# youthHan/HVRNet

Measured on AMD Instinct MI355X. Metric: VID frames/sec, R101 Faster-RCNN+HVR, 1000x600, 300 props, T=15, higher is better.
Workload: dtype bf16; 1 GPU; configs[2]: faster_rcnn_r101_hrnmp_c5 inference, clip mode; frames_per_window=15, proposals_per_frame=300, input=3x600x1000 padded to 608x1008, parallelism=dp1 independent clips, no collectives, windows_in_flight=4, clips_per_graph=1, key_frame_detections=300

## Files before the change

### hvrnet_amd/csrc/bigtile.hip

```cpp
#include <cstdlib>
#include <type_traits>
#include "common.h"
#include "gemm_params.h"

namespace hvr {

namespace {

constexpr int BG_BN = 256, BG_NT = 512, BG_WN = 4, BG_FN = 4, BG_WCOLS = BG_FN * 16;
constexpr int BG_B_SLOTS = BG_BN * 8 / BG_NT;

__device__ __forceinline__ uint32_t bg_lds_off(const void* p) {
  return (uint32_t)(uintptr_t)(const __attribute__((address_space(3))) char*)p;
}
template <int OFF> __device__ __forceinline__ uint4 bg_read128(uint32_t addr) {
  uint4 v;
  asm volatile("ds_read_b128 %0, %1 offset:%2" : "=v"(v) : "v"(addr), "n"(OFF));
  return v;
}
template <typename T> __device__ __forceinline__ void bg_mma(const uint4& w, const uint4& x, f32x4& acc) {
  if constexpr (std::is_same<T, bf16_t>::value)
    acc = __builtin_amdgcn_mfma_f32_16x16x32_bf16(__builtin_bit_cast(bf16x8, w), __builtin_bit_cast(bf16x8, x), acc, 0, 0, 0);
  else
    acc = __builtin_amdgcn_mfma_f32_16x16x32_f16(__builtin_bit_cast(f16x8, w), __builtin_bit_cast(f16x8, x), acc, 0, 0, 0);
}
__device__ __forceinline__ void bg_load_lds16(const void* base, char* lds, unsigned voff, int soff) {
#if defined(__HIP_DEVICE_COMPILE__)
  const __amdgpu_buffer_rsrc_t rs = __builtin_amdgcn_make_buffer_rsrc(const_cast<void*>(base), 0, (int)0x80000000u, 0x00020000);
  __builtin_amdgcn_raw_ptr_buffer_load_lds(rs, (__attribute__((address_space(3))) void*)lds, 16, (int)voff, soff, 0, 0);
#else
  (void)base; (void)lds; (void)voff; (void)soff;
#endif
}

}

template <typename T, int FM0, int FM1>
__global__ __launch_bounds__(BG_NT) void big_tile_kernel(const GemmParams p) {
  constexpr bool SPLIT = std::is_same<T, f16s_t>::value;
  constexpr int EB = (int)sizeof(T), KSG = 128;
  constexpr int BKE = SPLIT ? 32 : 64;
  constexpr int BM = (FM0 + FM1) * 16;
  constexpr int A_BYTES = BM * 128, STAGE = A_BYTES + BG_BN * 128;
  constexpr int A_SLOTS = (BM * 8 + BG_NT - 1) / BG_NT;
  constexpr int LAST_WAVES = (BM * 8 - (A_SLOTS - 1) * BG_NT) / 64;
  extern __shared__ __attribute__((aligned(16))) char smem[];
  const int tid = threadIdx.x, lane = tid & 63;
  const int wave = __builtin_amdgcn_readfirstlane(tid >> 6);
  const int wm = wave / BG_WN, wn = wave % BG_WN;
  const int wrow0 = wm ? FM0 * 16 : 0;
  const int tiles_n = p.N / BG_BN, tiles_m = (p.M + BM - 1) / BM;
  const int total = tiles_m * tiles_n, nwg = (int)gridDim.x;
  auto tile_of = [&](int r) -> int {
    const int left = total - r * nwg, here = left < nwg ? left : nwg;
    return (int)blockIdx.x < here ? r * nwg + xcd_remap(blockIdx.x, here) : -1;
  };
#ifdef HVR_DBG_BG_CLK
  long long dbg_t[1 + 3 * 3];
  for (int q = 0; q < 10; ++q) dbg_t[q] = 0;
  dbg_t[0] = wall_clock64();
#endif

  const int l_row = tid >> 3, l_chunk = ((tid & 7) ^ (l_row & 7)) * 16;
  int a_bias = 0;
  if (p.conv) a_bias = (int)(((long)p.pad * p.W + p.pad) * p.Cin * EB);
  const char* const rs_a = (const char*)p.A - a_bias;
  const char* const rs_b = (const char*)p.B;
  const bool seg2 = p.s2 > 0;
  const int k1_steps = seg2 ? p.K1 / BKE : 0x7fffffff;
  const char* const rs_a2 = (const char*)p.A2;
  const bool is_conv = p.conv != 0;
  const int cCin = is_conv ? p.Cin : 0x40000000, cKW = is_conv ? p.KW : 1, cDil = is_conv ? p.dil : 0;
  const int cRowB = is_conv ? p.W * p.Cin * EB : 0, cPixB = is_conv ? p.Cin * EB : 0;

  constexpr bool SEG2 = !SPLIT;
  struct TileState { int a_off[A_SLOTS], a_off2[SEG2 ? A_SLOTS : 1], b_off[BG_B_SLOTS]; unsigned oob[A_SLOTS]; int m0, n0; };
  auto setup = [&](int tile, TileState& st) {
    const __attribute__((address_space(4))) GemmParams* kq =
        (const __attribute__((address_space(4))) GemmParams*)__builtin_amdgcn_kernarg_segment_ptr();
    asm volatile("" : "+s"(kq));
    const int pid_m = tile / tiles_n, pid_n = tile - pid_m * tiles_n;
    st.m0 = pid_m * BM;
    st.n0 = pid_n * BG_BN;
    int a_yx[A_SLOTS];
#pragma unroll
    for (int i = 0; i < A_SLOTS; ++i) {
      int m = st.m0 + i * 64 + l_row;
      m = m < kq->M ? m : kq->M - 1;
      if constexpr (SEG2) st.a_off2[i] = 0;
      if (kq->conv || (SEG2 && kq->s2 > 0)) {
        const int ox = m % kq->OW, t = m / kq->OW, oy = t % kq->OH, b = t / kq->OH;
        if (kq->conv) {
          const int iy = oy * kq->stride - kq->pad, ix = ox * kq->stride - kq->pad;
          a_yx[i] = (iy << 16) | (ix & 0xffff);
          st.a_off[i] = (int)((((long)b * kq->H + iy) * kq->W + ix) * (long)kq->Cin * EB) + l_chunk + (int)(((long)kq->pad * kq->W + kq->pad) * kq->Cin * EB);
        } else {
          a_yx[i] = 0;
          st.a_off[i] = (int)((long)m * kq->lda * EB) + l_chunk;
        }
        if constexpr (SEG2) if (kq->s2 > 0) st.a_off2[i] = (int)((((long)b * kq->H2 + oy * kq->s2) * kq->W2 + ox * kq->s2) * (long)(kq->K - kq->K1) * EB) + l_chunk;
      } else {
        a_yx[i] = 0;
        st.a_off[i] = (int)((long)m * kq->lda * EB) + l_chunk;
      }
    }
#pragma unroll
    for (int i = 0; i < BG_B_SLOTS; ++i) st.b_off[i] = (int)((long)(st.n0 + i * 64 + l_row) * kq->ldb * EB) + l_chunk;
#pragma unroll
    for (int i = 0; i < A_SLOTS; ++i) st.oob[i] = 0u;
    if (kq->conv != 0) {
      unsigned colbad[A_SLOTS];
#pragma unroll
      for (int i = 0; i < A_SLOTS; ++i) colbad[i] = 0u;
      for (int kx = 0, dx = 0; kx < kq->KW; ++kx, dx += kq->dil) {
#pragma unroll
        for (int i = 0; i < A_SLOTS; ++i) colbad[i] |= (unsigned)((short)a_yx[i] + dx) < (unsigned)kq->W ? 0u : (1u << kx);
      }
      const unsigned all_kw = kq->KW >= 32 ? ~0u : (1u << kq->KW) - 1u;
      for (int ky = 0, dy = 0, sh = 0; ky < kq->KH; ++ky, dy += kq->dil, sh += kq->KW) {
#pragma unroll
        for (int i = 0; i < A_SLOTS; ++i) st.oob[i] |= ((unsigned)((a_yx[i] >> 16) + dy) < (unsigned)kq->H ? colbad[i] : all_kw) << sh;
      }
    }
  };
  TileState cs, ns;
  int cur_tile = tile_of(0), nxt_tile = tile_of(1);
  setup(cur_tile, cs);
  setup(nxt_tile >= 0 ? nxt_tile : cur_tile, ns);

  int a_koff = 0, b_koff = 0, kt_load = 0, t_cin0 = 0, t_kx = 0, t_ky = 0, t_tap = 0;
  const int nk_real = p.K / BKE;
  auto tap_next = [&](int adv, bool rst) {
    kt_load += adv;
    b_koff += adv * KSG;
    t_cin0 += adv * BKE;
    const bool w1 = t_cin0 >= cCin;
    t_cin0 = w1 ? 0 : t_cin0;
    t_tap += w1 ? 1 : 0;
    t_kx += w1 ? 1 : 0;
    const bool w2 = t_kx >= cKW;
    t_kx = w2 ? 0 : t_kx;
    t_ky += w2 ? 1 : 0;
    const int wmask = -(int)w1;
    a_koff = ((t_ky * cDil * cRowB + t_kx * cDil * cPixB) & wmask) | ((a_koff + adv * KSG) & ~wmask);
    const int keep = rst ? 0 : -1;
    kt_load &= keep; b_koff &= keep; t_cin0 &= keep; t_kx &= keep; t_ky &= keep; t_tap &= keep; a_koff &= keep;
  };
  auto dma_a = [&](auto I, char* stage, bool nx) {
    constexpr int i = decltype(I)::value;
    if (i < A_SLOTS - 1 || wave < LAST_WAVES) {
      const unsigned ao = (unsigned)(nx ? ns.a_off[i] : cs.a_off[i]), ob = nx ? ns.oob[i] : cs.oob[i];
      const unsigned voff = ao | ((ob >> (t_tap & 31)) << 31);
      if constexpr (SEG2) {
        const bool s2 = kt_load >= k1_steps;
        const char* const base = s2 ? rs_a2 : rs_a;
        const unsigned vo = s2 ? (unsigned)(nx ? ns.a_off2[i] : cs.a_off2[i]) : voff;
        const int so = s2 ? (kt_load - k1_steps) * KSG : a_koff;
        bg_load_lds16(base, stage + (i * BG_NT + wave * 64) * 16, vo, __builtin_amdgcn_readfirstlane(so));
      } else {
        bg_load_lds16(rs_a, stage + (i * BG_NT + wave * 64) * 16, voff, __builtin_amdgcn_readfirstlane(a_koff));
      }
    }
  };
  auto dma_b = [&](auto I, char* stage, bool nx) {
    constexpr int i = decltype(I)::value;
    bg_load_lds16(rs_b, stage + A_BYTES + (i * BG_NT + wave * 64) * 16, (unsigned)(nx ? ns.b_off[i] : cs.b_off[i]), __builtin_amdgcn_readfirstlane(b_koff));
  };

  static_for<A_SLOTS>([&](auto I) { dma_a(I, smem, false); });
  static_for<BG_B_SLOTS>([&](auto I) { dma_b(I, smem, false); });

  auto body = [&](auto FMC) {
  constexpr int FM = decltype(FMC)::value;
  int par = 0;
  for (int round = 0;; ++round) {
  const bool has_next = nxt_tile >= 0;
  const int m0 = cs.m0, n0 = cs.n0;
  f32x4 acc[FM][BG_FN];
#pragma unroll
  for (int i = 0; i < FM; ++i)
#pragma unroll
    for (int j = 0; j < BG_FN; ++j) acc[i][j] = f32x4{0.f, 0.f, 0.f, 0.f};

  const int frag_row = lane & 15, frag_grp = lane >> 4, swz = lane & 7;
  const uint32_t a_lane = bg_lds_off(smem) + (wrow0 + frag_row) * 128 + ((frag_grp ^ swz) * 16);
  const uint32_t b_lane = bg_lds_off(smem) + A_BYTES + (wn * BG_WCOLS + frag_row) * 128 + ((frag_grp ^ swz) * 16);

  const int nk = nk_real;
  if (round == 0) asm volatile("s_waitcnt vmcnt(0)" ::: "memory");
  __builtin_amdgcn_s_barrier();
#ifdef HVR_DBG_BG_CLK
  if (round < 3) dbg_t[1 + 3 * round] = wall_clock64();
#endif

  {
    constexpr int G0 = (FM + 1) / 2;
    constexpr int DMA_TOTAL = A_SLOTS + BG_B_SLOTS, DMA_FIRST = DMA_TOTAL / 2;
    auto kloop = [&](auto WMC) __attribute__((always_inline)) {
    constexpr int wmc = decltype(WMC)::value;
    constexpr int dma_ph = wmc ? 0 : 1;
    if constexpr (wmc != 0) __builtin_amdgcn_s_barrier();
    for (int kt = 0; kt < nk; ++kt) {
      const uint32_t soff = (uint32_t)((kt + par) & 1) * STAGE;
      char* nxt = smem + ((kt + 1 + par) & 1) * STAGE;
      const uint32_t a0 = a_lane + soff, b0 = b_lane + soff;
      uint4 kb[BG_FN], qa[G0];
      const bool last = kt + 1 >= nk, pre = last && has_next;
      tap_next(last ? 0 : 1, pre);
      constexpr int NPH = SPLIT ? 6 : 4;
      static_for<NPH>([&](auto PH) {
        constexpr int ph = decltype(PH)::value, term = ph >> 1, r0 = (ph & 1) ? G0 : 0, nr = (ph & 1) ? FM - G0 : G0;
        constexpr bool b_lo = term == 1, a_lo = SPLIT ? term == 2 : term == 1;
        if constexpr ((ph & 1) == 0)
          static_for<BG_FN>([&](auto J) { kb[decltype(J)::value] = bg_read128<decltype(J)::value * 2048>(b_lo ? (b0 ^ 64u) : b0); });
        static_for<nr>([&](auto R) {
          constexpr int r = decltype(R)::value;
          qa[r] = bg_read128<(r0 + r) * 2048>(a_lo ? (a0 ^ 64u) : a0);
        });
        __builtin_amdgcn_sched_barrier(0);
        if constexpr (ph < 3) {
          if constexpr (dma_ph == ph) {
            static_for<DMA_FIRST>([&](auto D) {
              constexpr int d = decltype(D)::value;
              if constexpr (d < A_SLOTS) dma_a(std::integral_constant<int, d>{}, nxt, pre);
              else dma_b(std::integral_constant<int, d - A_SLOTS>{}, nxt, pre);
            });
          } else if constexpr (dma_ph + 1 == ph) {
            static_for<DMA_TOTAL - DMA_FIRST>([&](auto D) {
              constexpr int d = DMA_FIRST + decltype(D)::value;
              if constexpr (d < A_SLOTS) dma_a(std::integral_constant<int, d>{}, nxt, pre);
              else dma_b(std::integral_constant<int, d - A_SLOTS>{}, nxt, pre);
            });
          }
        }
        if constexpr (ph == NPH - 1) {
          if constexpr (wmc != 0) asm volatile("s_waitcnt vmcnt(0)" ::: "memory");
        }
        __builtin_amdgcn_sched_barrier(0);
        __builtin_amdgcn_s_barrier();
        asm volatile("s_waitcnt lgkmcnt(0)" ::: "memory");
        __builtin_amdgcn_sched_barrier(0);
        __builtin_amdgcn_s_setprio(1);
        static_for<nr>([&](auto R) {
          constexpr int r = decltype(R)::value;
          static_for<BG_FN>([&](auto J) { bg_mma<T>(kb[decltype(J)::value], qa[r], acc[r0 + r][decltype(J)::value]); });
        });
        __builtin_amdgcn_s_setprio(0);
        __builtin_amdgcn_sched_barrier(0);
        if constexpr (ph == NPH - 1) {
          if constexpr (wmc == 0) asm volatile("s_waitcnt vmcnt(0)" ::: "memory");
        }
        __builtin_amdgcn_s_barrier();
      });
    }
    if constexpr (wmc == 0) __builtin_amdgcn_s_barrier();
    };
    int wsel = wave;
    asm volatile("" : "+s"(wsel));
    if (wsel >= BG_WN) kloop(std::integral_constant<int, 1>{});
    else kloop(std::integral_constant<int, 0>{});
  }
#ifdef HVR_DBG_BG_CLK
  if (round < 3) dbg_t[2 + 3 * round] = wall_clock64();
#endif

  char* const epi_base = smem + ((nk - 1 + par) & 1) * STAGE;
  const __attribute__((address_space(4))) GemmParams* kp =
      (const __attribute__((address_space(4))) GemmParams*)__builtin_amdgcn_kernarg_segment_ptr();
  asm volatile("" : "+s"(kp));
  if constexpr (SPLIT) {
    int etid = threadIdx.x;
    asm volatile("" : "+v"(etid));
    const int el = etid & 63, erow = el & 15, egrp = el >> 4;
    constexpr int SP = 256;
    char* stg = epi_base + wave * (16 * SP);
    float bias[BG_FN][4];
#pragma unroll
    for (int j = 0; j < BG_FN; ++j) {
      const int n = n0 + wn * BG_WCOLS + j * 16 + egrp * 4;
      if (kp->bias) {
        const float4 b = *reinterpret_cast<const float4*>(kp->bias + n);
        bias[j][0] = b.x; bias[j][1] = b.y; bias[j][2] = b.z; bias[j][3] = b.w;
        if (kp->beta != 0.f) {
#pragma unroll
          for (int r = 0; r < 4; ++r) bias[j][r] *= kp->beta;
        }
      } else {
        bias[j][0] = bias[j][1] = bias[j][2] = bias[j][3] = 0.f;
      }
    }
    auto slot = [&](int j, int plane) {
      const int piece = (j >> 1) * 8 + plane * 4 + 2 * (j & 1) + (egrp >> 1);
      return stg + erow * SP + ((piece ^ erow) << 4) + (egrp & 1) * 8;
    };
    const bool has_res = kp->resid != nullptr;
    const long col_bytes = split_col_bytes(n0 + wn * BG_WCOLS);
    auto load_res = [&](int i, uint4 (&rv)[4]) {
#pragma unroll
      for (int it = 0; it < 4; ++it) {
        const int q = it * 64 + el, row = q >> 4, pc = q & 15;
        int m = m0 + wrow0 + i * 16 + row;
        m = m < kp->M ? m : kp->M - 1;
        rv[it] = *reinterpret_cast<const uint4*>((const char*)kp->resid + (long)m * kp->ldr * 4 + col_bytes + pc * 16);
      }
    };
    uint4 rnext[4] = {make_uint4(0u, 0u, 0u, 0u), make_uint4(0u, 0u, 0u, 0u), make_uint4(0u, 0u, 0u, 0u), make_uint4(0u, 0u, 0u, 0u)};
    if (has_res) load_res(0, rnext);
    asm volatile("s_waitcnt lgkmcnt(0)" ::: "memory");
    __builtin_amdgcn_s_barrier();
#pragma unroll
    for (int i = 0; i < FM; ++i) {
      if (has_res) {
#pragma unroll
        for (int it = 0; it < 4; ++it) {
          const int q = it * 64 + el, row = q >> 4, pc = q & 15;
          *reinterpret_cast<uint4*>(stg + row * SP + ((pc ^ row) << 4)) = rnext[it];
        }
        if (i + 1 < FM) load_res(i + 1, rnext);
      }
#pragma unroll
      for (int j = 0; j < BG_FN; ++j) {
        f32x4 v = acc[i][j];
        if (kp->alpha != 0.f) v *= kp->alpha;
        float e[4];
#pragma unroll
        for (int r = 0; r < 4; ++r) e[r] = v[r] + bias[j][r];
        char* sh = slot(j, 0);
        char* sl = slot(j, 1);
        if (has_res) {
          const uint2 rh = *reinterpret_cast<const uint2*>(sh), rl = *reinterpret_cast<const uint2*>(sl);
          float r0_, r1_, r2_, r3_;
          merge2(rh.x, rl.x, r0_, r1_);
          merge2(rh.y, rl.y, r2_, r3_);
          e[0] += r0_; e[1] += r1_; e[2] += r2_; e[3] += r3_;
        }
        if (kp->relu) {
#pragma unroll
          for (int r = 0; r < 4; ++r) e[r] = fmaxf(e[r], 0.f);
        }
        uint2 oh, ol;
        split2(e[0], e[1], oh.x, ol.x);
        split2(e[2], e[3], oh.y, ol.y);
        *reinterpret_cast<uint2*>(sh) = oh;
        *reinterpret_cast<uint2*>(sl) = ol;
      }
#pragma unroll
      for (int it = 0; it < 4; ++it) {
        const int q = it * 64 + el, row = q >> 4, pc = q & 15;
        const int m = m0 + wrow0 + i * 16 + row;
        const uint4 v = *reinterpret_cast<const uint4*>(stg + row * SP + ((pc ^ row) << 4));
        if (m < kp->M) *reinterpret_cast<uint4*>((char*)kp->C + (long)m * kp->ldc * 4 + col_bytes + pc * 16) = v;
      }
    }
  } else
  {
    int etid = threadIdx.x;
    asm volatile("" : "+v"(etid));
    const int el = etid & 63, erow = el & 15, egrp = el >> 4;
    constexpr int SPITCH = BG_WCOLS * 2;
    char* stg = epi_base + wave * (16 * SPITCH);
    const int wr_lane = erow * SPITCH + (((egrp & 1) ^ (erow >> 3)) << 3);
    float bias[BG_FN][4];
#pragma unroll
    for (int j = 0; j < BG_FN; ++j) {
      const int n = n0 + wn * BG_WCOLS + j * 16 + egrp * 4;
      if (kp->bias) {
        const float4 b = *reinterpret_cast<const float4*>(kp->bias + n);
        bias[j][0] = b.x; bias[j][1] = b.y; bias[j][2] = b.z; bias[j][3] = b.w;
      } else {
        bias[j][0] = bias[j][1] = bias[j][2] = bias[j][3] = 0.f;
      }
    }
    const int st_row = el >> 3, st_chunk = el & 7;
    const bool has_res = kp->resid != nullptr;
    auto load_res = [&](int i, uint4 (&rv)[2]) {
#pragma unroll
      for (int h = 0; h < 2; ++h) {
        int m = m0 + wrow0 + i * 16 + h * 8 + st_row;
        m = m < kp->M ? m : kp->M - 1;
        rv[h] = *reinterpret_cast<const uint4*>((const unsigned short*)kp->resid + (long)m * kp->ldr + n0 + wn * BG_WCOLS + st_chunk * 8);
      }
    };
    uint4 rnext[2] = {make_uint4(0u, 0u, 0u, 0u), make_uint4(0u, 0u, 0u, 0u)};
    if (has_res) load_res(0, rnext);
    asm volatile("s_waitcnt lgkmcnt(0)" ::: "memory");
    __builtin_amdgcn_s_barrier();
#pragma unroll
    for (int i = 0; i < FM; ++i) {
      if (has_res) {
#pragma unroll
        for (int h = 0; h < 2; ++h) {
          const uint4 v = h ? make_uint4(rnext[h].z, rnext[h].w, rnext[h].x, rnext[h].y) : rnext[h];
          *reinterpret_cast<uint4*>(stg + (h * 8 + st_row) * SPITCH + ((st_chunk ^ st_row) << 4)) = v;
        }
        if (i + 1 < FM) load_res(i + 1, rnext);
      }
#pragma unroll
      for (int j = 0; j < BG_FN; ++j) {
        char* slot = stg + wr_lane + (((2 * j + (egrp >> 1)) ^ (erow & 7)) << 4);
        float e[4];
#pragma unroll
        for (int r = 0; r < 4; ++r) e[r] = acc[i][j][r] + bias[j][r];
        if (has_res) {
          const uint2 rr = *reinterpret_cast<const uint2*>(slot);
          float r0_, r1_, r2_, r3_;
          unpack2<T>(rr.x, r0_, r1_);
          unpack2<T>(rr.y, r2_, r3_);
          e[0] += r0_; e[1] += r1_; e[2] += r2_; e[3] += r3_;
        }
        if (kp->relu) {
#pragma unroll
          for (int r = 0; r < 4; ++r) e[r] = fmaxf(e[r], 0.f);
        }
        *reinterpret_cast<uint2*>(slot) = make_uint2(pack2<T>(e[0], e[1]), pack2<T>(e[2], e[3]));
      }
#pragma unroll
      for (int h = 0; h < 2; ++h) {
        const int row = h * 8 + st_row, m = m0 + wrow0 + i * 16 + row;
        uint4 v = *reinterpret_cast<const uint4*>(stg + row * SPITCH + ((st_chunk ^ st_row) << 4));
        if (h) v = make_uint4(v.z, v.w, v.x, v.y);
        if (m < kp->M) *reinterpret_cast<uint4*>((unsigned short*)kp->C + (long)m * kp->ldc + n0 + wn * BG_WCOLS + st_chunk * 8) = v;
      }
    }
  }
#ifdef HVR_DBG_BG_CLK
  if (round < 3) dbg_t[3 + 3 * round] = wall_clock64();
#endif
  if (!has_next) break;
  par = (par + nk) & 1;
  cs = ns;
  cur_tile = nxt_tile;
  nxt_tile = tile_of(round + 2);
  if (nxt_tile >= 0) setup(nxt_tile, ns);
  }
#ifdef HVR_DBG_BG_CLK
  asm volatile("s_waitcnt vmcnt(0)" ::: "memory");
  {
    const long long t_end = wall_clock64();
    if (threadIdx.x == 0 && (blockIdx.x % 5) == 0)
      printf("BGCLK wg %d t0 %lld | tile0 loop %lld..%lld epi %lld | tile1 loop %lld..%lld epi %lld | tile2 loop %lld..%lld epi %lld | drained %lld\n", (int)blockIdx.x, dbg_t[0],
             dbg_t[1] ? dbg_t[1] - dbg_t[0] : 0, dbg_t[2] ? dbg_t[2] - dbg_t[0] : 0, dbg_t[3] ? dbg_t[3] - dbg_t[0] : 0,
             dbg_t[4] ? dbg_t[4] - dbg_t[0] : 0, dbg_t[5] ? dbg_t[5] - dbg_t[0] : 0, dbg_t[6] ? dbg_t[6] - dbg_t[0] : 0,
             dbg_t[7] ? dbg_t[7] - dbg_t[0] : 0, dbg_t[8] ? dbg_t[8] - dbg_t[0] : 0, dbg_t[9] ? dbg_t[9] - dbg_t[0] : 0, t_end - dbg_t[0]);
  }
#endif
  };
  if constexpr (FM0 == FM1) {
    body(std::integral_constant<int, FM0>{});
  } else {
    if (wm == 0) body(std::integral_constant<int, FM0>{});
    else body(std::integral_constant<int, FM1>{});
  }
}

bool bigtile_supported(const GemmParams& p, bool throughput) {
  const bool split = p.dtype == DT_F16S;
  if ((p.dtype != DT_BF16 && p.dtype != DT_F16 && !split) || !p.staging || p.out_f32 || p.ksplit_steps > 0) return false;
  const int es = split ? 4 : 2, bke = split ? 32 : 64, row_al = split ? 32 : 8;
  if (p.s2 > 0 && (split || p.conv || p.K1 % 64 || (p.K - p.K1) % 64 || p.K1 < 64 || (reinterpret_cast<uintptr_t>(p.A2) & 15) ||
                   (long)p.M * (p.K - p.K1) * 2 >= (1L << 31))) return false;
  if (p.N % BG_BN || p.K % bke || p.ldc % row_al || p.lda % row_al || p.ldb % row_al) return false;
  if (p.resid && (p.ldr % row_al || (reinterpret_cast<uintptr_t>(p.resid) & (split ? 127 : 15)))) return false;
  if (split && ((reinterpret_cast<uintptr_t>(p.A) | reinterpret_cast<uintptr_t>(p.B) | reinterpret_cast<uintptr_t>(p.C)) & 127)) return false;
  if (p.tile_hint != kBigForce && (p.K < 256 || (p.resid && throughput && !split))) return false;
  if (p.conv && (p.Cin % bke || p.KH * p.KW > 32)) return false;
  const uintptr_t al = reinterpret_cast<uintptr_t>(p.A) | reinterpret_cast<uintptr_t>(p.B) | reinterpret_cast<uintptr_t>(p.C) |
                       reinterpret_cast<uintptr_t>(p.bias);
  if (al & 15) return false;
  if ((long)p.N * p.ldb * es >= (1L << 31)) return false;
  const long tiles = (long)((p.M + 287) / 288) * (p.N / BG_BN);
  static const int on = std::getenv("HVR_BIGTILE") ? std::atoi(std::getenv("HVR_BIGTILE")) : 1;
  constexpr int min_alone = 170;
  constexpr int min_shared = 96;
  if (p.tile_hint == kBigForce) return true;
  return on && tiles >= (throughput ? min_shared : min_alone) && tiles <= 4096;
}

template <typename T, int FM0, int FM1>
static hipError_t launch_bigtile(const GemmParams& p, hipStream_t stream) {
  constexpr int BM = (FM0 + FM1) * 16, lds = 2 * (BM + BG_BN) * 128;
  auto kern = big_tile_kernel<T, FM0, FM1>;
  static std::atomic<unsigned> attr_set_dev{0};
  per_device_once(attr_set_dev, [&] {
    (void)hipFuncSetAttribute(reinterpret_cast<const void*>(kern), hipFuncAttributeMaxDynamicSharedMemorySize, lds);
  });
  const int tiles = ((p.M + BM - 1) / BM) * (p.N / BG_BN);
  static const int nper = std::getenv("HVR_BIGTILE_WGS") ? std::atoi(std::getenv("HVR_BIGTILE_WGS")) : 256;
  const int grid = nper > 0 && tiles > nper ? nper : tiles;
  hipLaunchKernelGGL(kern, dim3(grid), dim3(BG_NT), lds, stream, p);
  return hipGetLastError();
}

hipError_t run_bigtile(const GemmParams& p, hipStream_t stream) {
  if (p.dtype == DT_F16S) return launch_bigtile<f16s_t, 9, 9>(p, stream);
  if (p.dtype == DT_F16) return launch_bigtile<f16_t, 9, 9>(p, stream);
  return launch_bigtile<bf16_t, 9, 9>(p, stream);
}

}
```

### hvrnet_amd/csrc/capi.hip

```cpp
#include "../../include/hvr_hip.h"

#include <cmath>
#include <cstdarg>
#include <cstdio>
#include <cstdlib>
#include <cstring>
#include <string>

#include "common.h"
#include "gemm_params.h"
#include "relation_bt.h"

namespace hvr {
hipError_t run_transpose_pad(const void*, void*, int, int, long, long, int, hipStream_t);
hipError_t run_zero_fill(void*, size_t, hipStream_t);
hipError_t run_pack_conv_weights_multi(const void*, int, long, int, hipStream_t);
hipError_t run_transpose_multi(const void*, int, int, hipStream_t);
hipError_t run_im2col_t(const void*, void*, int, int, int, int, int, int, int, int, int, int, long, hipStream_t);
hipError_t run_relu_bwd_t(const void*, const void*, void*, void*, int, int, long, hipStream_t);
hipError_t run_splitk_reduce(const float*, float*, int, int, long, int, hipStream_t);
hipError_t run_unpack_conv_wgrads_multi(const void*, int, long, int, hipStream_t);
hipError_t run_splitk_reduce_bf16(const float*, void*, int, int, long, int, hipStream_t);
hipError_t run_splitk_reduce_f16(const float*, void*, int, int, long, int, hipStream_t);
hipError_t run_splitk_reduce_half_batched(const float*, void*, int, int, long, int, int, int, long, long, hipStream_t);
hipError_t run_splitk_reduce_epi_bf16(const float*, void*, int, int, long, int, const float*, const void*, long, int, hipStream_t);
hipError_t run_relation_normalize(void*, const float*, const float*, int, int, long, int, float, hipStream_t);
hipError_t run_relu_bwd(const void*, const void*, void*, long, int, hipStream_t);
hipError_t run_im2col_nhwc(const void*, void*, int, int, int, int, int, int, int, int, int, int, int, hipStream_t);
hipError_t run_scale_rows(const void*, const float*, void*, int, long, int, hipStream_t);
hipError_t run_sgd_step(float*, const float*, float*, long, float, float, float, float, float, float*, int, hipStream_t);
hipError_t run_colsum(const void*, float*, int, int, long, int, float*, hipStream_t);
int colsum_slices(int M, int N);
size_t sgd_workspace_bytes();
hipError_t run_pack_conv_weight(const float*, const float*, void*, int, int, int, int, hipStream_t);
hipError_t run_unpack_conv_wgrad(const float*, const float*, float*, int, int, int, int, hipStream_t);
hipError_t run_det_loss(const float*, int, int, int, int, const long long*, const float*, const float*, const float*, int, float, float,
                        float, float*, float*, const int*, hipStream_t);
size_t assign_workspace_bytes(int n, int k);
hipError_t run_max_iou_assign(const float*, int, int, const float*, int, const uint8_t*, float, float, float, float, long long*, float*,
                              void*, hipStream_t);
hipError_t run_sample(const long long*, const float*, int, int, int, float, long long*, int*, hipStream_t);
hipError_t run_box_targets(const float*, int, int, const float*, const long long*, const long long*, const long long*, const int*, int,
                           const float*, const float*, float, int, long long*, float*, float*, float*, hipStream_t);
hipError_t run_rpn_loss(const float*, int, int, int, const long long*, const float*, const float*, const float*, const int*, float, float*,
                        float*, hipStream_t);
hipError_t run_ce_rows(const float*, int, int, int, const long long*, int, float*, hipStream_t);
hipError_t run_triplet_margin(const void*, long, const void*, long, int, int, int, const long long*, const long long*, const long long*, int,
                              float, int, float*, float*, float*, float*, hipStream_t);
hipError_t run_ingest(const uint8_t*, int, int, long, float*, int, int, int, int, const float*, const float*, int, int, hipStream_t);
size_t tta_merge_proposals_workspace_bytes(int A, int T, int mx);
hipError_t run_tta_merge_proposals(const float*, const int*, int, int, int, const float*, const float*, const int*, float, int, float*, int*, void*,
                                   hipStream_t);
hipError_t run_tta_map_rois(const float*, int, int, int, const float*, const float*, const int*, float*, hipStream_t);
hipError_t run_tta_merge_dets(const float*, const float*, int, int, int, const float*, const float*, const int*, float*, float*, hipStream_t);
hipError_t run_mining_argreduce(const float*, int, int, long, const long long*, const long long*, long long*, hipStream_t);
hipError_t run_relation_dscore(const void*, const void*, const void*, const void*, void*, int, long, int, long, long, float, int, hipStream_t);
hipError_t run_im2col_stem(const float*, void*, int, int, int, int, int, int, int, hipStream_t);
hipError_t run_maxpool3x3s2(const void*, void*, int, int, int, int, int, int, int, hipStream_t);
hipError_t run_cast(const void*, void*, long, int, int, float, hipStream_t);
hipError_t run_permute(const void*, void*, int, int, int, int, int, int, hipStream_t);
hipError_t run_det_decode(const float*, int, int, int, int, const float*, int, const float*, const float*, float, float,
                          float, float, float*, float*, hipStream_t);
hipError_t run_roi_align_fwd(const void*, const float*, void*, int, int, int, int, int, int, int, float, int, int, int,
                             hipStream_t);
hipError_t run_roi_align_bwd(const float*, const float*, float*, int, int, int, int, int, int, float, int, int, hipStream_t);
hipError_t run_deform_im2col(const void*, const float*, void*, int, int, int, int, int, int, int, int, int, int, int, int, long, int, int,
                             hipStream_t);
size_t nms_workspace_bytes(int P, int n);
hipError_t run_nms_batched(const float*, int, int, float, int, int, int, long long*, int*, void*, hipStream_t, int band = 0,
                           int* band_done = nullptr);
hipError_t run_rpn_select(const void*, const void*, long, long, float*, const RpnParams&, int, hipStream_t);
hipError_t run_rpn_select_wide(const void*, const void*, long, long, float*, const RpnParams&, void*, hipStream_t);
size_t rpn_wide_workspace_bytes(int T, long n_anchor);
int rpn_wide_max_frames(int set);
int* rpn_wide_done_flags(void* wws, int T);
hipError_t run_rpn_gather(const float*, const long long*, const int*, int, int, int, int, int, float*, int*, hipStream_t);
hipError_t run_multiclass_nms(const float*, const float*, int, int, float, float, int, float*, long long*, int*, void*,
                              hipStream_t);
size_t multiclass_nms_workspace_bytes(int R, int ncls);
hipError_t run_soft_nms(const float*, int, float, int, float, float, float*, long long*, int*, hipStream_t);
hipError_t run_multiclass_soft_nms(const float*, const float*, int, int, int, float, float, int, float, float, int, float*, long long*, int*,
                                   void*, hipStream_t);
size_t multiclass_soft_nms_workspace_bytes(int P, int R, int ncls);
hipError_t run_seq_nms(const float*, const float*, int, const int*, int, int, int, float, float, float, int, int, float*, long long*, int*, int*,
                       int*, float*, int*, int, void*, int, hipStream_t);
size_t seq_nms_workspace_bytes(int P, int F, int R, int ncls, int tubes);
hipError_t run_stem_fused(const float*, const void*, const float*, void*, int, int, int, int, hipStream_t);
}

using namespace hvr;

static thread_local std::string g_err;

static int fail(int code, const char* fmt, ...) {
  char buf[512];
  va_list ap;
  va_start(ap, fmt);
  vsnprintf(buf, sizeof buf, fmt, ap);
  va_end(ap);
  g_err = buf;
  return code;
}
static int check_launch(hipError_t e, const char* what) {
  if (e == hipSuccess) return HVR_OK;
  if (e == hipErrorInvalidValue) return fail(HVR_EUNSUPPORTED, "%s: shape outside the implemented envelope", what);
  return fail(HVR_ELAUNCH, "%s: %s", what, hipGetErrorString(e));
}
static inline size_t align256(size_t b) { return (b + 255) & ~(size_t)255; }
static inline int elem_size(int dtype) { return (dtype == HVR_BF16 || dtype == HVR_F16) ? 2 : 4; }
static inline int kstep_elems(int dtype) { return (dtype == HVR_F32 || dtype == HVR_F16S) ? 32 : 64; }
static inline bool valid_dtype(int dtype) { return dtype >= HVR_F32 && dtype <= HVR_F16S; }
static inline bool aligned128(const void* p) { return (reinterpret_cast<uintptr_t>(p) & 127) == 0; }
static inline bool aligned16(const void* p) { return (reinterpret_cast<uintptr_t>(p) & 15) == 0; }

extern "C" {

int hvr_abi_version(void) { return 6; }
const char* hvr_last_error(void) { return g_err.c_str(); }

static int fill_linear(GemmParams& p, const void* A, const void* B, void* C, int M, int N, int K, long lda, long ldb,
                       long ldc, int dtype, int staging) {
  std::memset(&p, 0, sizeof p);
  if (!valid_dtype(dtype)) return fail(HVR_EINVAL, "dtype %d is none of HVR_F32 / HVR_BF16 / HVR_F16 / HVR_F16S", dtype);
  const int bke = kstep_elems(dtype);
  if (!A || !B || !C) return fail(HVR_EINVAL, "null operand pointer");
  if (M <= 0 || N <= 0 || K <= 0) return fail(HVR_EINVAL, "empty problem M=%d N=%d K=%d", M, N, K);
  if (K % bke) return fail(HVR_EINVAL, "K=%d is not a multiple of the %d-element K-step", K, bke);
  if (N % 4) return fail(HVR_EINVAL, "N=%d is not a multiple of 4", N);
  if (!aligned16(A) || !aligned16(B) || !aligned16(C)) return fail(HVR_EINVAL, "operands must be 16-byte aligned");
  if (dtype == HVR_F16S && (lda % 32 || ldb % 32 || !aligned128(A) || !aligned128(B)))
    return fail(HVR_EINVAL, "split-half operands need 128-byte aligned bases and row pitches that are multiples of 32 elements");
  const long es = elem_size(dtype);
  if ((long)M * lda * es >= (1L << 31) || (long)N * ldb * es >= (1L << 31))
    return fail(HVR_EUNSUPPORTED, "operand of 2 GiB or more (M=%d lda=%ld N=%d ldb=%ld)", M, lda, N, ldb);
  p.A = A; p.B = B; p.C = C;
  p.M = M; p.N = N; p.K = K;
  p.lda = lda; p.ldb = ldb; p.ldc = ldc;
  p.dtype = dtype;
  p.staging = staging ? 1 : 0;
  return HVR_OK;
}

static int fewrow_mode() {
  static const int on = std::getenv("HVR_CONV_SPLITK") ? std::atoi(std::getenv("HVR_CONV_SPLITK")) : 1;
  return on;
}
static int fewrow_slices(const GemmParams& p) {
  const int on = fewrow_mode();
  constexpr int target = 512, mink = 8, minper = 4;
  if (!on || p.dtype != DT_BF16 || !p.staging || p.out_f32 || p.tile_hint != 0) return 1;
  if (p.N % 8 || p.ldc % 8 || (p.resid && p.ldr % 8) || !aligned16(p.C) || (p.resid && !aligned16(p.resid)) || (p.bias && !aligned16(p.bias))) return 1;
  const long tiles = (long)((p.M + 127) / 128) * ((p.N + 63) / 64);
  const int ksteps = p.K / 64;
  if (tiles > 160 || ksteps < mink) return 1;
  long s = (target + tiles / 2) / tiles;
  if (s > ksteps / minper) s = ksteps / minper;
  return s < 2 ? 1 : (int)s;
}

static hipError_t run_fewrow_split(const GemmParams& p, int slices, void* ws, hipStream_t stream) {
  GemmParams q = p;
  const int ksteps = p.K / 64;
  q.ksplit_steps = (ksteps + slices - 1) / slices;
  q.ksplit_count = (ksteps + q.ksplit_steps - 1) / q.ksplit_steps;
  q.csplit_bytes = (long)p.M * p.N * 4;
  q.C = ws; q.ldc = p.N; q.out_f32 = 1;
  q.bias = nullptr; q.resid = nullptr; q.relu = 0;
  q.tile_hint = 2;
  hipError_t e = run_tile_op(q, EPI_LINEAR, stream);
  if (e == hipSuccess) e = run_splitk_reduce_epi_bf16((const float*)ws, p.C, p.M, p.N, p.ldc, q.ksplit_count, p.bias, p.resid, p.ldr, p.relu, stream);
  return e;
}

static int gemm_params(const hvr_gemm_desc* d, GemmParams& p) {
  if (!d) return fail(HVR_EINVAL, "null descriptor");
  int rc = fill_linear(p, d->A, d->B, d->C, d->M, d->N, d->K, d->lda, d->ldb, d->ldc, d->dtype, d->staging);
  if (rc) return rc;
  const int es = elem_size(d->dtype);
  if ((d->lda * es) % 16 || (d->ldb * es) % 16) return fail(HVR_EINVAL, "lda/ldb rows must be 16-byte multiples");
  if ((d->ldc * (d->out_f32 ? 4 : es)) % 8) return fail(HVR_EINVAL, "ldc rows must be 8-byte multiples");
  if (d->dtype == HVR_F16S) {
    if (!d->out_f32 && (d->N % 8 || d->ldc % 32 || !aligned128(d->C))) return fail(HVR_EINVAL, "split-half output: N %% 8 == 0, ldc %% 32 == 0, 128-byte aligned C");
    if (d->resid && (d->N % 8 || d->ldr % 32 || !aligned128(d->resid))) return fail(HVR_EINVAL, "split-half residual: N %% 8 == 0, ldr %% 32 == 0, 128-byte aligned");
  }
  p.bias = d->bias; p.resid = d->resid; p.ldr = d->ldr; p.relu = d->relu; p.out_f32 = d->out_f32;
  p.tile_hint = d->tile_hint;
  p.alpha = d->alpha; p.beta = d->beta;
  return 0;
}

size_t hvr_gemm_fewrow_workspace_bytes(const hvr_gemm_desc* d) {
  GemmParams p;
  if (gemm_params(d, p)) return 0;
  const int s = fewrow_slices(p);
  return s > 1 ? (size_t)s * p.M * p.N * 4 : 0;
}

int hvr_gemm(const hvr_gemm_desc* d, void* stream) {
  GemmParams p;
  const int rc = gemm_params(d, p);
  if (rc) return rc;
  int hint = d->tile_hint;
  if (hint == kBigForce) {
    if (!bigtile_supported(p, true)) return fail(HVR_EUNSUPPORTED, "the big-tile kernel takes bf16 products with N %% 256 == 0 and K %% 64 == 0");
    return check_launch(run_bigtile(p, (hipStream_t)stream), "hvr_gemm(big tile)");
  }
  if (hint == kBigHint || hint == 0) {
    const bool thr = hint == kBigHint;
    p.tile_hint = hint = 0;
    if (bigtile_supported(p, thr)) return check_launch(run_bigtile(p, (hipStream_t)stream), "hvr_gemm(big tile)");
  }
  if (d->tile_hint == kPcHint128 || d->tile_hint == kPcHint256) {
    if (!pc_supported(p, EPI_LINEAR)) return fail(HVR_EUNSUPPORTED, "the producer / consumer tile kernel takes aligned bf16 operands with N %% 8 == 0");
    return check_launch(run_pc(p, EPI_LINEAR, d->tile_hint == kPcHint256 ? 256 : 128, (hipStream_t)stream), "hvr_gemm (pc)");
  }
  if (hint == 0 && d->K >= 8192 && pc_supported(p, EPI_LINEAR)) {
    const long tiles = (long)((d->M + 143) / 144) * ((d->N + 127) / 128);
    if (tiles > 192 && tiles <= 256) return check_launch(run_pc(p, EPI_LINEAR, 128, (hipStream_t)stream), "hvr_gemm (pc)");
  }
  const int slices = fewrow_slices(p);
  if (slices > 1 && d->ws && aligned16(d->ws) && d->ws_bytes >= (size_t)slices * p.M * p.N * 4) {
    if (fewrow_mode() == 1 && kpar_supported(p)) return check_launch(run_kpar(p, (hipStream_t)stream), "hvr_gemm(K-parallel waves)");
    return check_launch(run_fewrow_split(p, slices, d->ws, (hipStream_t)stream), "hvr_gemm(split-K)");
  }
  return check_launch(run_tile_op(p, EPI_LINEAR, (hipStream_t)stream), "hvr_gemm");
}

static int splitk_slices(int M, int N, int K, int dtype) {
  const long tiles = (long)((M + 127) / 128) * ((N + 127) / 128);
  if (dtype == HVR_F16S) return 1;
  const int ksteps = K / kstep_elems(dtype);
  if (tiles >= 192 || ksteps < 32) return 1;
  long s = (512 + tiles - 1) / tiles;
  if (s > ksteps / 8) s = ksteps / 8;
  if (s > 64) s = 64;
  return s < 2 ? 1 : (int)s;
}

size_t hvr_gemm_splitk_workspace_bytes(int M, int N, int K, int dtype) {
  if (M <= 0 || N <= 0 || K <= 0 || !valid_dtype(dtype)) return 0;
  const int s = splitk_slices(M, N, K, dtype);
  return s > 1 ? (size_t)s * M * N * 4 : 0;
}

int hvr_gemm_splitk(const hvr_gemm_desc* d, void* ws, size_t ws_bytes, void* stream) {
  if (!d) return fail(HVR_EINVAL, "null descriptor");
  if (d->bias || d->resid || d->relu) return fail(HVR_EINVAL, "split-K products have no epilogue (bias / residual / ReLU)");
  if (d->dtype != HVR_F32 && !d->out_f32) return fail(HVR_EINVAL, "split-K products are f32 (set out_f32)");
  GemmParams p;
  int rc = fill_linear(p, d->A, d->B, d->C, d->M, d->N, d->K, d->lda, d->ldb, d->ldc, d->dtype, d->staging);
  if (rc) return rc;
  const int es = elem_size(d->dtype);
  if ((d->lda * es) % 16 || (d->ldb * es) % 16) return fail(HVR_EINVAL, "lda/ldb rows must be 16-byte multiples");
  if ((d->ldc * 4) % 8) return fail(HVR_EINVAL, "ldc rows must be 8-byte multiples");
  p.out_f32 = d->out_f32;
  p.tile_hint = d->tile_hint;
  const int slices = splitk_slices(d->M, d->N, d->K, d->dtype);
  if (slices <= 1) return check_launch(run_tile_op(p, EPI_LINEAR, (hipStream_t)stream), "hvr_gemm_splitk");
  const size_t need = (size_t)slices * d->M * d->N * 4;
  if (!ws || ws_bytes < need || !aligned16(ws)) return fail(HVR_EINVAL, "split-K workspace too small (%zu < %zu) or unaligned", ws_bytes, need);
  const int ksteps = d->K / kstep_elems(d->dtype);
  p.ksplit_steps = (ksteps + slices - 1) / slices;
  p.ksplit_count = (ksteps + p.ksplit_steps - 1) / p.ksplit_steps;
  p.csplit_bytes = (long)d->M * d->N * 4;
  p.C = ws;
  p.ldc = d->N;
  hipError_t e = run_tile_op(p, EPI_LINEAR, (hipStream_t)stream);
  if (e == hipSuccess) e = run_splitk_reduce((const float*)ws, (float*)d->C, d->M, d->N, d->ldc, p.ksplit_count, (hipStream_t)stream);
  return check_launch(e, "hvr_gemm_splitk");
}

static int splitk_slices_batched(int M, int N, int K, int dtype, int count) {
  const long tiles = (long)((M + 127) / 128) * ((N + 127) / 128) * count;
  if (dtype == HVR_F16S) return 1;
  const int ksteps = K / kstep_elems(dtype);
  if (tiles >= 384 || ksteps < 32) return 1;
  long s = (512 + tiles - 1) / tiles;
  if (s > ksteps / 8) s = ksteps / 8;
  if (s > 64) s = 64;
  return s < 2 ? 1 : (int)s;
}

size_t hvr_gemm_splitk_batched_workspace_bytes(int M, int N, int K, int dtype, int count) {
  if (M <= 0 || N <= 0 || K <= 0 || count <= 0 || !valid_dtype(dtype)) return 0;
  const int s = splitk_slices_batched(M, N, K, dtype, count);
  return s > 1 ? (size_t)s * count * M * N * 4 : 0;
}

int hvr_gemm_splitk_batched(const hvr_gemm_desc* d, int count, int64_t stride_a, int64_t stride_b, int64_t stride_c, void* ws, size_t ws_bytes,
                            void* stream) {
  if (!d || count <= 0) return fail(HVR_EINVAL, "null descriptor / count <= 0");
  if (d->bias || d->resid || d->relu) return fail(HVR_EINVAL, "split-K products have no epilogue (bias / residual / ReLU)");
  if (d->dtype != HVR_F32 && !d->out_f32) return fail(HVR_EINVAL, "split-K products are f32 (set out_f32)");
  if (d->dtype == HVR_F16S) return fail(HVR_EUNSUPPORTED, "batched split-K products take f32 / bf16 / half operands");
  GemmParams p;
  int rc = fill_linear(p, d->A, d->B, d->C, d->M, d->N, d->K, d->lda, d->ldb, d->ldc, d->dtype, d->staging);
  if (rc) return rc;
  const int es = elem_size(d->dtype);
  if ((d->lda * es) % 16 || (d->ldb * es) % 16 || (stride_a * es) % 16 || (stride_b * es) % 16) return fail(HVR_EINVAL, "lda / ldb rows and the problem strides must be 16-byte multiples");
  if ((d->ldc * 4) % 8 || (stride_c * 4) % 16) return fail(HVR_EINVAL, "ldc rows must be 8-byte, stride_c 16-byte multiples");
  if (stride_a * es >= (1L << 31) || stride_b * es >= (1L << 31)) return fail(HVR_EUNSUPPORTED, "one problem's operands must stay below 2 GiB");
  p.out_f32 = d->out_f32;
  p.tile_hint = d->tile_hint;
  p.batch = count;
  p.gs_a = stride_a * es; p.gs_b = stride_b * es; p.gs_c = stride_c * 4;
  const int slices = splitk_slices_batched(d->M, d->N, d->K, d->dtype, count);
  if (slices <= 1) return check_launch(run_tile_op(p, EPI_LINEAR, (hipStream_t)stream), "hvr_gemm_splitk_batched");
  if (d->ldc != d->N || stride_c != (int64_t)d->M * d->N) return fail(HVR_EINVAL, "the sliced form writes one contiguous [count][M][N] output (ldc = N, stride_c = M * N)");
  const size_t need = (size_t)slices * count * d->M * d->N * 4;
  if (!ws || ws_bytes < need || !aligned16(ws)) return fail(HVR_EINVAL, "split-K workspace too small (%zu < %zu) or unaligned", ws_bytes, need);
  if ((long)count * d->M > 0x7fffffffL) return fail(HVR_EUNSUPPORTED, "too many output rows");
  const int ksteps = d->K / kstep_elems(d->dtype);
  p.ksplit_steps = (ksteps + slices - 1) / slices;
  p.ksplit_count = (ksteps + p.ksplit_steps - 1) / p.ksplit_steps;
  p.csplit_bytes = (long)count * d->M * d->N * 4;
  p.gs_c = (long)d->M * d->N * 4;
  p.C = ws;
  p.ldc = d->N;
  hipError_t e = run_tile_op(p, EPI_LINEAR, (hipStream_t)stream);
  if (e == hipSuccess) e = run_splitk_reduce((const float*)ws, (float*)d->C, count * d->M, d->N, d->N, p.ksplit_count, (hipStream_t)stream);
  return check_launch(e, "hvr_gemm_splitk_batched");
}

static int expand_enabled() {
  static const int on = std::getenv("HVR_EXPAND") ? std::atoi(std::getenv("HVR_EXPAND")) : 1;
  return on;
}

static int conv_params(const hvr_conv_desc* d, GemmParams& p, int& path) {
  if (!d) return fail(HVR_EINVAL, "null descriptor");
  const int OH = (d->H + 2 * d->pad - d->dil * (d->KH - 1) - 1) / d->stride + 1;
  const int OW = (d->W + 2 * d->pad - d->dil * (d->KW - 1) - 1) / d->stride + 1;
  if (OH <= 0 || OW <= 0) return fail(HVR_EINVAL, "empty conv output %dx%d", OH, OW);
  if (!valid_dtype(d->dtype)) return fail(HVR_EINVAL, "bad dtype %d", d->dtype);
  const int bke = kstep_elems(d->dtype);
  if (d->Cin % bke) return fail(HVR_EINVAL, "Cin=%d is not a multiple of %d", d->Cin, bke);
  if (d->dtype == HVR_F16S && !d->out_f32 && (d->Cout % 32 || !aligned128(d->y))) return fail(HVR_EINVAL, "split-half conv output: Cout %% 32 == 0, 128-byte aligned y");
  if (d->dtype == HVR_F16S && d->resid && (d->Cout % 32 || !aligned128(d->resid))) return fail(HVR_EINVAL, "split-half conv residual: Cout %% 32 == 0, 128-byte aligned");
  const long M = (long)d->B * OH * OW;
  if (M > 0x7fffffffL) return fail(HVR_EUNSUPPORTED, "too many output pixels");
  if ((long)d->B * d->H * d->W * d->Cin * (long)elem_size(d->dtype) >= (1L << 31))
    return fail(HVR_EUNSUPPORTED, "conv input of 2 GiB or more");
  const int K = d->KH * d->KW * d->Cin;
  int rc = fill_linear(p, d->x, d->w, d->y, (int)M, d->Cout, K, d->Cin, K, d->Cout, d->dtype, d->staging);
  if (rc) return rc;
  const bool pointwise = d->KH == 1 && d->KW == 1 && d->stride == 1 && d->pad == 0;
  if (!pointwise) {
    if (!d->zero) return fail(HVR_EINVAL, "conv needs the zero page");
    p.conv = 1; p.H = d->H; p.W = d->W; p.Cin = d->Cin; p.OH = OH; p.OW = OW; p.KH = d->KH; p.KW = d->KW;
    p.stride = d->stride; p.pad = d->pad; p.dil = d->dil; p.zero = d->zero;
  }
  p.bias = d->bias; p.resid = d->resid; p.ldr = d->Cout; p.relu = d->relu; p.out_f32 = d->out_f32;
  p.tile_hint = d->tile_hint;
  p.alpha = d->alpha; p.beta = d->beta;
  if (pointwise) p.zero = d->zero;
  const int use_expand = expand_enabled();
  if (p.tile_hint == kBigForce) {
    path = 0;
    return 0;
  }
  const bool hint0 = p.tile_hint == 0 || p.tile_hint == kBigHint;
  bool big_first = false;
  if (hint0 && pointwise) {
    GemmParams q = p;
    q.tile_hint = 0;
    big_first = bigtile_supported(q, p.tile_hint == kBigHint);
    if (big_first && p.resid && p.K == 256 && p.dtype != DT_F16S && p.M >= 65536 && expand_supported(p)) big_first = false;
  }
  path = (pointwise && (expand_supported(p) || expand_split_supported(p)) &&
          (p.tile_hint == kExpandHint || (hint0 && use_expand && p.resid && p.N >= 2 * p.K && !big_first))) ? 1 : 0;
  if (p.tile_hint == kExpandHint) p.tile_hint = 0;
  static const int use_c3 = std::getenv("HVR_CONV3") ? std::atoi(std::getenv("HVR_CONV3")) : 1;
  if (path == 0 && hint0 && use_c3 && conv3x3_c64_supported(p)) path = 2;
  if (path != 0 && p.tile_hint == kBigHint) p.tile_hint = 0;
  return 0;
}

size_t hvr_conv2d_splitk_workspace_bytes(const hvr_conv_desc* d) {
  GemmParams p;
  int path = 0;
  if (conv_params(d, p, path)) return 0;
  const int s = (path == 0 ? fewrow_slices(p) : 1);
  return s > 1 ? (size_t)s * p.M * p.N * 4 : 0;
}

int hvr_conv2d_nhwc(const hvr_conv_desc* d, void* stream) {
  GemmParams p;
  int path = 0;
  const int rc = conv_params(d, p, path);
  if (rc) return rc;
  if (path == 1) return check_launch(p.dtype == DT_F16S ? run_expand_split(p, (hipStream_t)stream) : run_expand(p, (hipStream_t)stream), "hvr_conv2d_nhwc(expand)");
  if (path == 2) return check_launch(run_conv3x3_c64(p, (hipStream_t)stream), "hvr_conv2d_nhwc(conv3x3_c64)");
  if (path == 0 && d->tile_hint == kBigForce) {
    if (!bigtile_supported(p, true)) return fail(HVR_EUNSUPPORTED, "the big-tile kernel takes bf16 convs with Cout %% 256 == 0 and Cin %% 64 == 0");
    return check_launch(run_bigtile(p, (hipStream_t)stream), "hvr_conv2d_nhwc(big tile)");
  }
  if (path == 0 && d->tile_hint == kTwoLevelHint) {
    p.tile_hint = 0;
    if (two_level_supported(p)) return check_launch(run_tile_op(p, EPI_LINEAR2, (hipStream_t)stream), "hvr_conv2d_nhwc(two-level)");
  }
  if (path == 0 && (d->tile_hint == kBigHint || d->tile_hint == 0 || d->tile_hint == kTwoLevelHint)) {
    p.tile_hint = 0;
    if (bigtile_supported(p, d->tile_hint == kBigHint)) return check_launch(run_bigtile(p, (hipStream_t)stream), "hvr_conv2d_nhwc(big tile)");
  }
  const int slices = (path == 0 ? fewrow_slices(p) : 1);
  if (slices > 1 && d->ws && aligned16(d->ws) && d->ws_bytes >= (size_t)slices * p.M * p.N * 4) {
    if (fewrow_mode() == 1 && kpar_supported(p)) return check_launch(run_kpar(p, (hipStream_t)stream), "hvr_conv2d_nhwc(K-parallel waves)");
    const hipError_t e = run_fewrow_split(p, slices, d->ws, (hipStream_t)stream);
    return check_launch(e, "hvr_conv2d_nhwc(split-K)");
  }
  return check_launch(run_tile_op(p, EPI_LINEAR, (hipStream_t)stream), "hvr_conv2d_nhwc");
}

static int tail_params(const hvr_tail_desc* d, GemmParams& p) {
  if (!d) return fail(HVR_EINVAL, "null descriptor");
  if (d->dtype != HVR_BF16 && d->dtype != HVR_F16) return fail(HVR_EUNSUPPORTED, "hvr_bottleneck_tail takes bf16 or half operands");
  if (d->B <= 0 || d->OH <= 0 || d->OW <= 0 || d->stride2 <= 0) return fail(HVR_EINVAL, "empty tail problem");
  if ((d->OH - 1) * d->stride2 >= d->H2 || (d->OW - 1) * d->stride2 >= d->W2) return fail(HVR_EINVAL, "the sampled pixels fall outside x");
  const long M = (long)d->B * d->OH * d->OW;
  if (M > 0x7fffffffL) return fail(HVR_EUNSUPPORTED, "too many output pixels");
  const int K = d->C1 + d->C2;
  int rc = fill_linear(p, d->h, d->w, d->y, (int)M, d->Cout, K, d->C1, K, d->Cout, d->dtype, 1);
  if (rc) return rc;
  if (!d->x || !aligned16(d->x)) return fail(HVR_EINVAL, "x must be a 16-byte aligned device pointer");
  if ((long)d->B * d->H2 * d->W2 * d->C2 * 2 >= (1L << 31)) return fail(HVR_EUNSUPPORTED, "block input of 2 GiB or more");
  p.bias = d->bias; p.relu = d->relu;
  p.A2 = d->x; p.K1 = d->C1; p.H2 = d->H2; p.W2 = d->W2; p.s2 = d->stride2; p.OH = d->OH; p.OW = d->OW;
  return 0;
}

static bool tail_on_tile_engine(const GemmParams& p) {
  return (p.dtype == DT_BF16 || p.dtype == DT_F16) && p.K1 % 64 == 0 && (p.K - p.K1) % 64 == 0 && p.K1 >= 64 && p.K - p.K1 >= 64 && p.N % 8 == 0 && p.ldc % 8 == 0 &&
         (long)p.M * (p.K - p.K1) * 2 < (1L << 31);
}

int hvr_bottleneck_tail_supported(const hvr_tail_desc* d) {
  GemmParams p;
  if (tail_params(d, p)) return 0;
  return (expand_supported(p) || tail_on_tile_engine(p)) ? 1 : 0;
}

int hvr_bottleneck_tail(const hvr_tail_desc* d, void* stream) {
  GemmParams p;
  const int rc = tail_params(d, p);
  if (rc) return rc;
  if (expand_supported(p)) return check_launch(run_expand(p, (hipStream_t)stream), "hvr_bottleneck_tail");
  if (tail_on_tile_engine(p)) {
    if (bigtile_supported(p, false)) return check_launch(run_bigtile(p, (hipStream_t)stream), "hvr_bottleneck_tail(big tile)");
    return check_launch(run_tile_op(p, EPI_LINEAR, (hipStream_t)stream), "hvr_bottleneck_tail(tile engine)");
  }
  return fail(HVR_EUNSUPPORTED, "no fused tail kernel for C1=%d C2=%d Cout=%d", d->C1, d->C2, d->Cout);
}

static int tail_next_params(const hvr_tail_next_desc* d, GemmParams& p) {
  if (!d) return fail(HVR_EINVAL, "null descriptor");
  const hvr_tail_desc& t = d->tail;
  if (t.C2 > 0) {
    const int rc = tail_params(&t, p);
    if (rc) return rc;
  } else {
    if (t.dtype != HVR_BF16 && t.dtype != HVR_F16 && t.dtype != HVR_F16S)
      return fail(HVR_EUNSUPPORTED, "hvr_bottleneck_tail_next takes bf16, half or (identity form) split-half operands");
    if (t.B <= 0 || t.OH <= 0 || t.OW <= 0) return fail(HVR_EINVAL, "empty tail problem");
    const long M = (long)t.B * t.OH * t.OW;
    if (M > 0x7fffffffL) return fail(HVR_EUNSUPPORTED, "too many output pixels");
    const int rc = fill_linear(p, t.h, t.w, t.y, (int)M, t.Cout, t.C1, t.C1, t.C1, t.Cout, t.dtype, 1);
    if (rc) return rc;
    const bool split = t.dtype == HVR_F16S;
    if (!d->resid || !(split ? aligned128(d->resid) : aligned16(d->resid)))
      return fail(HVR_EINVAL, "an identity block needs its (16-byte aligned; split half: 128-byte aligned) residual map");
    if (split && (t.Cout % 32 || !aligned128(t.y))) return fail(HVR_EINVAL, "split-half tail: Cout %% 32 == 0, 128-byte aligned y");
    p.bias = t.bias; p.relu = t.relu; p.resid = d->resid; p.ldr = t.Cout;
    if (t.dtype == HVR_F16S) { p.alpha = d->alpha; p.beta = d->beta; }
  }
  if (!t.relu) return fail(HVR_EUNSUPPORTED, "the next block reads the activated output (relu = 1)");
  p.Wn = d->wn; p.bias_n = d->bias_n; p.Hn = d->hn; p.Cn = d->Cn;
  return 0;
}

int hvr_bottleneck_tail_next_supported(const hvr_tail_next_desc* d) {
  GemmParams p;
  if (tail_next_params(d, p)) return 0;
  return (expand_next_supported(p) || expand_split_next_supported(p)) ? 1 : 0;
}

int hvr_bottleneck_tail_next(const hvr_tail_next_desc* d, void* stream) {
  GemmParams p;
  const int rc = tail_next_params(d, p);
  if (rc) return rc;
  if (expand_split_next_supported(p)) return check_launch(run_expand_split(p, (hipStream_t)stream), "hvr_bottleneck_tail_next(split half)");
  if (!expand_next_supported(p))
    return fail(HVR_EUNSUPPORTED, "no fused tail + next conv kernel for C1=%d C2=%d Cout=%d Cn=%d", d->tail.C1, d->tail.C2, d->tail.Cout, d->Cn);
  return check_launch(run_expand(p, (hipStream_t)stream), "hvr_bottleneck_tail_next");
}

static int close_sampled_params(const hvr_close_sampled_desc* d, GemmParams& p) {
  if (!d) return fail(HVR_EINVAL, "null descriptor");
  if (!valid_dtype(d->dtype)) return fail(HVR_EINVAL, "bad dtype %d", d->dtype);
  if (d->B <= 0 || d->OH <= 0 || d->OW <= 0 || d->rstride <= 0 || d->RH <= 0 || d->RW <= 0) return fail(HVR_EINVAL, "empty sampled-close problem");
  if ((long)(d->OH - 1) * d->rstride >= d->RH || (long)(d->OW - 1) * d->rstride >= d->RW) return fail(HVR_EINVAL, "the sampled pixels fall outside resid");
  const long M = (long)d->B * d->OH * d->OW;
  if (M > 0x7fffffffL || (long)d->B * d->RH * d->RW > 0x7fffffffL) return fail(HVR_EUNSUPPORTED, "too many pixels");
  const int rc = fill_linear(p, d->h, d->w, d->y, (int)M, d->Cout, d->C1, d->C1, d->C1, d->Cout, d->dtype, 1);
  if (rc) return rc;
  const bool split = d->dtype == HVR_F16S;
  if (!d->resid || !(split ? aligned128(d->resid) : aligned16(d->resid)))
    return fail(HVR_EINVAL, "resid must be a 16-byte aligned (split half: 128-byte aligned) device pointer");
  if (split && (d->Cout % 32 || !aligned128(d->y))) return fail(HVR_EINVAL, "split-half sampled close: Cout %% 32 == 0, 128-byte aligned y");
  p.bias = d->bias; p.relu = d->relu; p.resid = d->resid; p.ldr = d->Cout;
  p.rs = d->rstride; p.RH = d->RH; p.RW = d->RW; p.OH = d->OH; p.OW = d->OW;
  if (split) { p.alpha = d->alpha; p.beta = d->beta; }
  return 0;
}

int hvr_bottleneck_close_sampled_supported(const hvr_close_sampled_desc* d) {
  GemmParams p;
  if (close_sampled_params(d, p)) return 0;
  return (expand_enabled() && p.N >= 2 * p.K && (expand_supported(p) || expand_split_supported(p))) ? 1 : 0;
}

int hvr_bottleneck_close_sampled(const hvr_close_sampled_desc* d, void* stream) {
  GemmParams p;
  const int rc = close_sampled_params(d, p);
  if (rc) return rc;
  if (expand_enabled() && p.N >= 2 * p.K) {
    if (expand_split_supported(p)) return check_launch(run_expand_split(p, (hipStream_t)stream), "hvr_bottleneck_close_sampled(split half)");
    if (expand_supported(p)) return check_launch(run_expand(p, (hipStream_t)stream), "hvr_bottleneck_close_sampled");
  }
  return fail(HVR_EUNSUPPORTED, "no sampled-residual closing kernel for C1=%d Cout=%d dtype=%d (%d output pixels)", d->C1, d->Cout, d->dtype, p.M);
}

int hvr_conv2d_path(const hvr_conv_desc* d) {
  GemmParams p;
  int path = 0;
  const int rc = conv_params(d, p, path);
  if (rc) return rc;
  if (path == 0 && (d->tile_hint == 0 || d->tile_hint == kBigHint)) {
    p.tile_hint = 0;
    if (bigtile_supported(p, d->tile_hint == kBigHint)) return 3;
  }
  return path;
}

int hvr_im2col_stem(const float* img, void* cols, int B, int H, int W, int KP, int dtype, void* stream) {
  if (!img || !cols || B <= 0) return fail(HVR_EINVAL, "bad stem arguments");
  if (dtype == HVR_F16S && (KP % 32 || !aligned128(cols))) return fail(HVR_EINVAL, "split-half patch rows: KP %% 32 == 0, 128-byte aligned");
  if (KP < 147 || KP % kstep_elems(dtype)) return fail(HVR_EINVAL, "KP=%d must be >= 147 and a K-step multiple", KP);
  const int OH = (H + 6 - 7) / 2 + 1, OW = (W + 6 - 7) / 2 + 1;
  return check_launch(run_im2col_stem(img, cols, B, H, W, OH, OW, KP, dtype, (hipStream_t)stream), "hvr_im2col_stem");
}

int hvr_stem_fused_dtype(const float* img, const void* wpk, const float* bias, void* out, int B, int H, int W, int dtype, void* stream) {
  if (!img || !wpk || !bias || !out || B <= 0 || H < 7 || W < 7) return fail(HVR_EINVAL, "bad fused-stem arguments");
  if (dtype != HVR_BF16 && dtype != HVR_F16 && dtype != HVR_F16S) return fail(HVR_EUNSUPPORTED, "the fused stem computes on bf16, half or split-half operands");
  if (!aligned16(wpk) || !aligned16(out) || !aligned16(bias)) return fail(HVR_EINVAL, "fused stem operands must be 16-byte aligned");
  if (dtype == HVR_F16S && !aligned128(out)) return fail(HVR_EINVAL, "split-half stem output must be 128-byte aligned");
  return check_launch(run_stem_fused(img, wpk, bias, out, B, H, W, dtype, (hipStream_t)stream), "hvr_stem_fused");
}
int hvr_stem_fused(const float* img, const void* wpk, const float* bias, void* out, int B, int H, int W, void* stream) {
  return hvr_stem_fused_dtype(img, wpk, bias, out, B, H, W, HVR_BF16, stream);
}

int hvr_maxpool3x3s2_nhwc(const void* x, void* y, int B, int H, int W, int C, int dtype, void* stream) {
  if (!x || !y || C % 4) return fail(HVR_EINVAL, "bad maxpool arguments (C %% 4 == 0 required)");
  if (dtype == HVR_F16S) return fail(HVR_EUNSUPPORTED, "max pooling runs on f32 / bf16 / half maps");
  const int OH = (H + 2 - 3) / 2 + 1, OW = (W + 2 - 3) / 2 + 1;
  return check_launch(run_maxpool3x3s2(x, y, B, H, W, C, OH, OW, dtype, (hipStream_t)stream), "hvr_maxpool3x3s2_nhwc");
}

static int env_tile(const char* name) {
  const char* v = std::getenv(name);
  return v ? std::atoi(v) : 0;
}
static inline long rel_ldp(int Mk) { return ((long)Mk + 127) / 128 * 128; }

static int apply_slice_blocks() { return 4; }
static int apply_slices(int Mq, int Mk, int D) {
  const long tiles = (long)((Mq + 127) / 128) * ((D + 127) / 128);
  const int nblk = (int)(rel_ldp(Mk) / 128);
  if (tiles >= 96 || nblk < 8 || D % 8) return 1;
  const int per = apply_slice_blocks();
  return (nblk + per - 1) / per;
}

static int relation_apply_pass(const void* P, const void* Vt, float* mstat, float* lstat, float* partial, void* O, int64_t ldo,
                               int Mq, int Mk, int D, long ldp, int nt, int dtype, int staging, hipStream_t s) {
  const bool two_byte = dtype == HVR_BF16 || dtype == HVR_F16;
  constexpr int tile_apply = 0, gm_apply = 1;
#ifdef HVR_DEBUG_KNOBS
  static const int dbg_ld0 = env_tile("HVR_DBG_LD0");
#endif
  GemmParams p;
  int rc;
  rc = fill_linear(p, P, Vt, O, Mq, D, (int)ldp, ldp, ldp, ldo, dtype, staging);
  if (rc) return rc;
  p.mstat = mstat; p.lstat = lstat; p.ntile = nt;
  p.tile_hint = tile_apply;
  p.group_m = gm_apply;
#ifdef HVR_DEBUG_KNOBS
  if (dbg_ld0 & 2) { p.lda = 0; p.ldb = 0; }
#endif
  const int slices = apply_slices(Mq, Mk, D);
  if (slices > 1 && tile_apply == 0 && (!two_byte || (ldo % 8 == 0 && aligned16(O)))) {
    const int steps_per_blk = two_byte ? 2 : 4;
    const int per = apply_slice_blocks();
    p.ksplit_steps = per * steps_per_blk;
    p.ksplit_count = slices;
    p.csplit_bytes = (long)Mq * D * 4;
    p.C = partial; p.ldc = D; p.out_f32 = two_byte ? 1 : 0;
    p.tile_hint = 1;
    hipError_t e = run_tile_op(p, EPI_APPLY, s);
    if (e == hipSuccess)
      e = dtype == HVR_BF16 ? run_splitk_reduce_bf16(partial, O, Mq, D, ldo, slices, s)
          : dtype == HVR_F16 ? run_splitk_reduce_f16(partial, O, Mq, D, ldo, slices, s) : run_splitk_reduce(partial, (float*)O, Mq, D, ldo, slices, s);
    return check_launch(e, "relation: apply (key slices)");
  }
  if (Mq >= 1024 && pc_supported(p, EPI_APPLY))
    return check_launch(run_pc(p, EPI_APPLY, 128, s), "relation: apply (pc)");
  return check_launch(run_tile_op(p, EPI_APPLY, s), "relation: apply");
}

constexpr int kNormalizeMaxBlocks = 128;
static int normalize_blocks_ok(int Mk, const char* what) {
  if (rel_ldp(Mk) / 128 > kNormalizeMaxBlocks)
    return fail(HVR_EUNSUPPORTED, "%s: Mk=%d exceeds the %d keys (%d blocks of 128) the normalising sweep supports", what, Mk,
                kNormalizeMaxBlocks * 128, kNormalizeMaxBlocks);
  return HVR_OK;
}
static bool split_normalizes(int Mq) {
  static const int split_normalize = std::getenv("HVR_SPLIT_NORMALIZE") ? std::atoi(std::getenv("HVR_SPLIT_NORMALIZE")) : -1;
  return split_normalize == 1 || (split_normalize < 0 && Mq >= 1024);
}

static int relation_split_tail(void* P, void* Vt, float* mstat, float* lstat, const void* V, int64_t ldv, void* O, int64_t ldo, int Mq,
                               int Mk, int D, long ldp, int nt, int staging, hipStream_t s) {
  constexpr int tile_apply_s = 0;
  int rc = V ? check_launch(run_transpose_pad(V, Vt, Mk, D, ldv, ldp, HVR_F16S, s), "relation: V transpose (split half)") : HVR_OK;
  if (rc) return rc;
  GemmParams p;
  rc = fill_linear(p, P, Vt, O, Mq, D, (int)ldp, ldp, ldp, ldo, HVR_F16S, staging);
  if (rc) return rc;
  p.alpha = 1.f / kSplitProbScale;
  p.mstat = mstat; p.lstat = lstat; p.ntile = nt;
  p.tile_hint = tile_apply_s;
#ifdef HVR_DEBUG_KNOBS
  static const int dbg_apply_s = env_tile("HVR_DBG_APPLY_S");
  if (dbg_apply_s) p.tile_hint = dbg_apply_s;
#endif
  if (split_normalizes(Mq)) {
    rc = check_launch(run_relation_normalize(P, mstat, lstat, Mq, nt, ldp, HVR_F16S, 1.f, s), "relation: normalise (split half)");
    if (rc) return rc;
    return check_launch(run_tile_op(p, EPI_LINEAR, s), "relation: apply (split half, plain product)");
  }
  return check_launch(run_tile_op(p, EPI_APPLY, s), "relation: apply (split half)");
}

size_t hvr_relation_workspace_bytes(int Mq, int Mk, int D, int dtype) {
  const long ldp = rel_ldp(Mk), nt = ldp / 128;
  const size_t es = elem_size(dtype);
  const int slices = apply_slices(Mq, Mk, D);
  return align256((size_t)Mq * ldp * es) + align256((size_t)D * ldp * es) + 2 * align256((size_t)Mq * nt * 4) +
         (slices > 1 ? align256((size_t)slices * Mq * D * 4) : 0);
}

int hvr_relation_fwd(const void* Q, int64_t ldq, const void* K, int64_t ldk, const void* V, int64_t ldv, void* O,
                     int64_t ldo, int Mq, int Mk, int D, float scale, int dtype, int staging, void* ws, size_t ws_bytes,
                     void* stream) {
  if (!Q || !K || !V || !O || !ws) return fail(HVR_EINVAL, "null pointer");
  if (Mq <= 0 || Mk <= 0) return fail(HVR_EINVAL, "empty relation Mq=%d Mk=%d", Mq, Mk);
  if (!(scale > 0.f)) return fail(HVR_EINVAL, "relation scale must be positive (the reference uses 1/sqrt(D)), got %g", (double)scale);
  if (ws_bytes < hvr_relation_workspace_bytes(Mq, Mk, D, dtype))
    return fail(HVR_EWORKSPACE, "relation workspace %zu < %zu", ws_bytes, hvr_relation_workspace_bytes(Mq, Mk, D, dtype));
  const long ldp = rel_ldp(Mk);
  const int nt = (int)(ldp / 128);
  const size_t es = elem_size(dtype);
  char* w = (char*)ws;
  void* P = w;                w += align256((size_t)Mq * ldp * es);
  void* Vt = w;               w += align256((size_t)D * ldp * es);
  float* mstat = (float*)w;   w += align256((size_t)Mq * nt * 4);
  float* lstat = (float*)w;   w += align256((size_t)Mq * nt * 4);
  float* partial = (float*)w;
  hipStream_t s = (hipStream_t)stream;

  GemmParams p;
  int rc;
  constexpr int tile_scores_s = 0;
  if (dtype == HVR_F16S) {
    if (ldv % 64 || !aligned128(V) || ldo % 32 || !aligned128(O) || D % 64) return fail(HVR_EINVAL, "split-half relation: D, ldv multiples of 64, ldo of 32, 128-byte aligned V / O");
    if (split_normalizes(Mq) && (rc = normalize_blocks_ok(Mk, "split-half relation"))) return rc;
    const bool bt = staging && scores_bt_supported(Mq, Mk, D, ldq, ldk, ldv, ldp, Q, K, V, P, Vt, 1, true);
    if (bt) {
      ScoresBTParams b;
      b.Q = (const bf16_t*)Q; b.K = (const bf16_t*)K; b.P = (bf16_t*)P; b.mstat = mstat; b.lstat = lstat;
      b.V = (const bf16_t*)V; b.Vt = (bf16_t*)Vt; b.Mq = Mq; b.Mk = Mk; b.D = D; b.ntile = nt;
      b.ldq = ldq; b.ldk = ldk; b.ldv = ldv; b.ldp = ldp; b.sl2 = scale * 1.4426950408889634f; b.f16 = 2;
      b.groups = 1; b.gs_q = b.gs_k = b.gs_v = b.gs_p = b.gs_vt = b.gs_stat = 0; b.int_max = 0;
      rc = check_launch(run_scores_bt(b, s), "relation: scores (split half, big tile)");
    } else {
      rc = fill_linear(p, Q, K, P, Mq, (Mk + 3) / 4 * 4, D, ldq, ldk, ldp, dtype, staging);
      if (rc) return rc;
      p.N = Mk; p.scale = scale; p.mstat = mstat; p.lstat = lstat; p.ntile = nt; p.group_m = 8;
      p.tile_hint = tile_scores_s;
      rc = check_launch(run_tile_op(p, EPI_SCORES, s), "relation: scores (split half)");
    }
    if (rc) return rc;
    return relation_split_tail(P, Vt, mstat, lstat, bt ? nullptr : V, ldv, O, ldo, Mq, Mk, D, ldp, nt, staging, s);
  }
  const bool two_byte = dtype == HVR_BF16 || dtype == HVR_F16;
  constexpr int tile_scores = 0, gm_scores = 8;
#ifdef HVR_DEBUG_KNOBS
  static const int dbg_ld0 = env_tile("HVR_DBG_LD0");
#endif
  const bool bt = two_byte && staging && scores_bt_supported(Mq, Mk, D, ldq, ldk, ldv, ldp, Q, K, V, P, Vt);
  if (bt) {
    ScoresBTParams b;
    b.Q = (const bf16_t*)Q; b.K = (const bf16_t*)K; b.P = (bf16_t*)P; b.mstat = mstat; b.lstat = lstat;
    b.V = (const bf16_t*)V; b.Vt = (bf16_t*)Vt; b.Mq = Mq; b.Mk = Mk; b.D = D; b.ntile = nt;
    b.ldq = ldq; b.ldk = ldk; b.ldv = ldv; b.ldp = ldp; b.sl2 = scale * 1.4426950408889634f; b.f16 = dtype == HVR_F16;
    b.groups = 1; b.gs_q = b.gs_k = b.gs_v = b.gs_p = b.gs_vt = b.gs_stat = 0; b.int_max = 0;
    rc = check_launch(run_scores_bt(b, s), "relation: scores (big tile)");
    if (rc) return rc;
  } else {
    const bool fold = two_byte && staging && Mq <= 1024 && D % 8 == 0 && ldv % 8 == 0 && aligned16(V) && aligned16(Vt);
    if (!fold) {
      rc = check_launch(run_transpose_pad(V, Vt, Mk, D, ldv, ldp, dtype, s), "relation: V transpose");
      if (rc) return rc;
    }
    rc = fill_linear(p, Q, K, P, Mq, (Mk + 3) / 4 * 4, D, ldq, ldk, ldp, dtype, staging);
    if (rc) return rc;
    if (fold) {
      p.tr_in = V; p.tr_out = Vt; p.tr_R = Mk; p.tr_C = D; p.tr_ldx = ldv; p.tr_ldt = ldp;
      const int score_tiles = ((Mq + 127) / 128) * ((Mk + 127) / 128);
      const int vt_tiles = ((D + 63) / 64) * (int)((ldp + 63) / 64);
      int nb = 256 - score_tiles % 256;
      if (nb < 64) nb += 256;
      p.tr_blocks = nb < vt_tiles ? nb : vt_tiles;
    }
    p.N = Mk;
    p.scale = scale; p.mstat = mstat; p.lstat = lstat; p.ntile = nt;
    p.tile_hint = tile_scores ? tile_scores : ((two_byte && staging && Mq <= 1024) ? 9 : 0);
    p.group_m = gm_scores;
#ifdef HVR_DEBUG_KNOBS
    if (dbg_ld0 & 1) { p.lda = 0; p.ldb = 0; }
#endif
    rc = check_launch(run_tile_op(p, EPI_SCORES, s), "relation: scores");
    if (rc) return rc;
  }
  return relation_apply_pass(P, Vt, mstat, lstat, partial, O, ldo, Mq, Mk, D, ldp, nt, dtype, staging, s);
}

size_t hvr_relation_grouped_workspace_bytes(int groups, int Mq, int Mk, int D, int dtype) {
  return (size_t)(groups > 0 ? groups : 0) * align256(hvr_relation_workspace_bytes(Mq, Mk, D, dtype));
}

// ... 717 lines not shown
```

### hvrnet_amd/csrc/gemm_params.h

```cpp
#pragma once
#include <hip/hip_runtime.h>

namespace hvr {

enum { EPI_LINEAR = 0, EPI_SCORES = 1, EPI_APPLY = 2, EPI_LINEAR2 = 3 };

struct RpnParams {
  int T, H, W, A, npre, n_anchor;
  int cls_pitch, reg_pitch;
  int stride;
  float img_h, img_w;
  float m[4], s[4];
  float max_ratio;
  float base[32][4];
};

struct GemmParams {
  const void* A;
  const void* B;
  void* C;
  int M, N, K;
  long lda, ldb, ldc;
  int dtype;
  int staging;
  int tile_hint;
  int conv, H, W, Cin, OH, OW, KH, KW, stride, pad, dil;
  const void* zero;
  const float* bias;
  const void* resid;
  long ldr;
  int relu, out_f32;
  float alpha;
  float beta;
  float scale;
  float* mstat;
  float* lstat;
  int ntile;
  int group_m;
  const void* A2;
  int K1, H2, W2, s2;
  int rs, RH, RW;
  const void* Wn;
  const float* bias_n;
  void* Hn;
  int Cn;
  int ksplit_steps, ksplit_count;
  long csplit_bytes;
  const void* tr_in;
  void* tr_out;
  int tr_R, tr_C, tr_blocks;
  long tr_ldx, tr_ldt;
  int batch;
  long gs_a, gs_b, gs_c, gs_stat, gs_tr_in, gs_tr_out;
};

struct TileShape { int bm, bn, wg_per_cu; float eff; };
constexpr int kNumTileShapes = 12;
constexpr int kNumBaseShapes = 5;
extern const TileShape kTileShapes[kNumTileShapes];
int choose_tile(const GemmParams& p, int epi);

hipError_t run_tile_op(const GemmParams& p, int epi, hipStream_t stream);
bool two_level_supported(const GemmParams& p);

constexpr int kExpandHint = kNumTileShapes + 1;
bool expand_supported(const GemmParams& p);
bool conv3x3_c64_supported(const GemmParams& p);
hipError_t run_conv3x3_c64(const GemmParams& p, hipStream_t stream);
hipError_t run_expand(const GemmParams& p, hipStream_t stream);
bool expand_next_supported(const GemmParams& p);
bool expand_split_supported(const GemmParams& p);
bool expand_split_next_supported(const GemmParams& p);
hipError_t run_expand_split(const GemmParams& p, hipStream_t stream);
constexpr int kPcHint128 = kNumTileShapes + 2, kPcHint256 = kNumTileShapes + 3;
bool pc_supported(const GemmParams& p, int epi);
constexpr int kBigHint = kNumTileShapes + 4, kBigForce = kNumTileShapes + 5, kTwoLevelHint = kNumTileShapes + 6;
constexpr int kTwoLevelSteps = 8;
bool bigtile_supported(const GemmParams& p, bool throughput);
hipError_t run_bigtile(const GemmParams& p, hipStream_t stream);
hipError_t run_pc(const GemmParams& p, int epi, int bn, hipStream_t stream);
bool kpar_supported(const GemmParams& p);
hipError_t run_kpar(const GemmParams& p, hipStream_t stream);

}
```

### hvrnet_amd/native.py

```python
import contextlib
import ctypes
import math
import os
import subprocess

import torch

_HERE = os.path.dirname(os.path.abspath(__file__))
LIB_PATH = os.path.join(_HERE, 'libhvr_hip.so')
HEADER_PATH = os.path.join(os.path.dirname(_HERE), 'include', 'hvr_hip.h')

HVR_F32, HVR_BF16, HVR_F16, HVR_F16S = 0, 1, 2, 3
ABI_VERSION = 6
SPLIT = torch.int32
COMPUTE_DTYPES = (torch.bfloat16, torch.float16, SPLIT, torch.float32)
DTYPE_NAMES = {torch.bfloat16: 'bf16', torch.float16: 'f16', SPLIT: 'f16x2', torch.float32: 'f32'}
LAYOUT_NCHW, LAYOUT_NHWC = 0, 1

STAGING = 1
TILE_HINT = 0


class HvrError(RuntimeError):
    pass


class GemmDesc(ctypes.Structure):
    _fields_ = [('A', ctypes.c_void_p), ('B', ctypes.c_void_p), ('C', ctypes.c_void_p),
                ('M', ctypes.c_int32), ('N', ctypes.c_int32), ('K', ctypes.c_int32),
                ('lda', ctypes.c_int64), ('ldb', ctypes.c_int64), ('ldc', ctypes.c_int64),
                ('bias', ctypes.c_void_p), ('resid', ctypes.c_void_p), ('ldr', ctypes.c_int64),
                ('relu', ctypes.c_int32), ('out_f32', ctypes.c_int32),
                ('dtype', ctypes.c_int32), ('staging', ctypes.c_int32), ('tile_hint', ctypes.c_int32),
                ('ws', ctypes.c_void_p), ('ws_bytes', ctypes.c_size_t), ('alpha', ctypes.c_float), ('beta', ctypes.c_float)]


class ConvDesc(ctypes.Structure):
    _fields_ = [('x', ctypes.c_void_p), ('w', ctypes.c_void_p), ('y', ctypes.c_void_p),
                ('B', ctypes.c_int32), ('H', ctypes.c_int32), ('W', ctypes.c_int32),
                ('Cin', ctypes.c_int32), ('Cout', ctypes.c_int32), ('KH', ctypes.c_int32),
                ('KW', ctypes.c_int32), ('stride', ctypes.c_int32), ('pad', ctypes.c_int32),
                ('dil', ctypes.c_int32),
                ('bias', ctypes.c_void_p), ('resid', ctypes.c_void_p),
                ('relu', ctypes.c_int32), ('out_f32', ctypes.c_int32),
                ('dtype', ctypes.c_int32), ('staging', ctypes.c_int32), ('tile_hint', ctypes.c_int32),
                ('zero', ctypes.c_void_p), ('ws', ctypes.c_void_p), ('ws_bytes', ctypes.c_size_t), ('alpha', ctypes.c_float),
                ('beta', ctypes.c_float)]


class TailDesc(ctypes.Structure):
    _fields_ = [('h', ctypes.c_void_p), ('x', ctypes.c_void_p), ('w', ctypes.c_void_p), ('y', ctypes.c_void_p),
                ('B', ctypes.c_int32), ('OH', ctypes.c_int32), ('OW', ctypes.c_int32), ('C1', ctypes.c_int32),
                ('H2', ctypes.c_int32), ('W2', ctypes.c_int32), ('C2', ctypes.c_int32), ('stride2', ctypes.c_int32),
                ('Cout', ctypes.c_int32), ('bias', ctypes.c_void_p), ('relu', ctypes.c_int32), ('dtype', ctypes.c_int32)]


class TailNextDesc(ctypes.Structure):
    _fields_ = [('tail', TailDesc), ('resid', ctypes.c_void_p), ('wn', ctypes.c_void_p), ('bias_n', ctypes.c_void_p),
                ('hn', ctypes.c_void_p), ('Cn', ctypes.c_int32), ('alpha', ctypes.c_float), ('beta', ctypes.c_float)]


class CloseSampledDesc(ctypes.Structure):
    _fields_ = [('h', ctypes.c_void_p), ('w', ctypes.c_void_p), ('resid', ctypes.c_void_p), ('y', ctypes.c_void_p),
                ('B', ctypes.c_int32), ('OH', ctypes.c_int32), ('OW', ctypes.c_int32), ('C1', ctypes.c_int32),
                ('Cout', ctypes.c_int32), ('RH', ctypes.c_int32), ('RW', ctypes.c_int32), ('rstride', ctypes.c_int32),
                ('bias', ctypes.c_void_p), ('relu', ctypes.c_int32), ('dtype', ctypes.c_int32),
                ('alpha', ctypes.c_float), ('beta', ctypes.c_float)]


class RpnDesc(ctypes.Structure):
    _fields_ = [('cls', ctypes.c_void_p), ('reg', ctypes.c_void_p),
                ('T', ctypes.c_int32), ('H', ctypes.c_int32), ('W', ctypes.c_int32),
                ('A', ctypes.c_int32), ('anchor_stride', ctypes.c_int32),
                ('base_anchors', ctypes.c_void_p), ('means', ctypes.c_void_p), ('stds', ctypes.c_void_p),
                ('img_h', ctypes.c_float), ('img_w', ctypes.c_float), ('wh_ratio_clip', ctypes.c_float),
                ('nms_pre', ctypes.c_int32), ('nms_post', ctypes.c_int32), ('max_num', ctypes.c_int32),
                ('nms_thr', ctypes.c_float),
                ('proposals', ctypes.c_void_p), ('counts', ctypes.c_void_p),
                ('cls_pitch', ctypes.c_int32), ('reg_pitch', ctypes.c_int32)]


_vp, _i, _f, _i64, _sz = ctypes.c_void_p, ctypes.c_int, ctypes.c_float, ctypes.c_int64, ctypes.c_size_t
SYMBOLS = {
    'hvr_abi_version': (_i, []),
    'hvr_last_error': (ctypes.c_char_p, []),
    'hvr_gemm': (_i, [ctypes.POINTER(GemmDesc), _vp]),
    'hvr_gemm_fewrow_workspace_bytes': (_sz, [ctypes.POINTER(GemmDesc)]),
    'hvr_gemm_splitk_workspace_bytes': (_sz, [_i, _i, _i, _i]),
    'hvr_gemm_splitk': (_i, [ctypes.POINTER(GemmDesc), _vp, _sz, _vp]),
    'hvr_gemm_splitk_batched_workspace_bytes': (_sz, [_i, _i, _i, _i, _i]),
    'hvr_gemm_splitk_batched': (_i, [ctypes.POINTER(GemmDesc), _i, _i64, _i64, _i64, _vp, _sz, _vp]),
    'hvr_conv2d_nhwc': (_i, [ctypes.POINTER(ConvDesc), _vp]),
    'hvr_conv2d_path': (_i, [ctypes.POINTER(ConvDesc)]),
    'hvr_conv2d_splitk_workspace_bytes': (_sz, [ctypes.POINTER(ConvDesc)]),
    'hvr_bottleneck_tail': (_i, [ctypes.POINTER(TailDesc), _vp]),
    'hvr_bottleneck_tail_supported': (_i, [ctypes.POINTER(TailDesc)]),
    'hvr_bottleneck_tail_next': (_i, [ctypes.POINTER(TailNextDesc), _vp]),
    'hvr_bottleneck_tail_next_supported': (_i, [ctypes.POINTER(TailNextDesc)]),
    'hvr_bottleneck_close_sampled': (_i, [ctypes.POINTER(CloseSampledDesc), _vp]),
    'hvr_bottleneck_close_sampled_supported': (_i, [ctypes.POINTER(CloseSampledDesc)]),
    'hvr_im2col_stem': (_i, [_vp, _vp, _i, _i, _i, _i, _i, _vp]),
    'hvr_maxpool3x3s2_nhwc': (_i, [_vp, _vp, _i, _i, _i, _i, _i, _vp]),
    'hvr_stem_fused': (_i, [_vp, _vp, _vp, _vp, _i, _i, _i, _vp]),
    'hvr_stem_fused_dtype': (_i, [_vp, _vp, _vp, _vp, _i, _i, _i, _i, _vp]),
    'hvr_relation_workspace_bytes': (_sz, [_i, _i, _i, _i]),
    'hvr_relation_fwd': (_i, [_vp, _i64, _vp, _i64, _vp, _i64, _vp, _i64, _i, _i, _i, _f, _i, _i, _vp, _sz, _vp]),
    'hvr_relation_grouped_workspace_bytes': (_sz, [_i, _i, _i, _i, _i]),
    'hvr_relation_fwd_grouped': (_i, [_vp, _i64, _i64, _vp, _i64, _i64, _vp, _i64, _i64, _vp, _i64, _i64, _i, _i, _i, _i, _f, _i, _i, _i, _vp, _sz, _vp]),
    'hvr_relation_probs_workspace_bytes': (_sz, [_i, _i]),
    'hvr_relation_probs': (_i, [_vp, _i64, _vp, _i64, _vp, _i64, _i, _i, _i, _f, _i, _i, _vp, _sz, _vp]),
    'hvr_relation_dscore': (_i, [_vp, _vp, _vp, _i64, _vp, _i64, _vp, _i, _i64, _i, _f, _i, _vp]),
    'hvr_relu_bwd': (_i, [_vp, _vp, _vp, _i64, _i, _vp]),
    'hvr_im2col_nhwc': (_i, [_vp, _vp, _i, _i, _i, _i, _i, _i, _i, _i, _i, _vp]),
    'hvr_im2col_t': (_i, [_vp, _vp, _i64, _i, _i, _i, _i, _i, _i, _i, _i, _i, _vp]),
    'hvr_relu_bwd_t': (_i, [_vp, _vp, _vp, _vp, _i64, _i, _i, _i, _vp]),
    'hvr_scale_rows': (_i, [_vp, _vp, _vp, _i, _i64, _i, _vp]),
    'hvr_sgd_workspace_bytes': (_sz, []),
    'hvr_sgd_step': (_i, [_vp, _vp, _vp, _i64, _f, _f, _f, _f, _f, _vp, _sz, _i, _vp]),
    'hvr_colsum_workspace_bytes': (_sz, [_i, _i]),
    'hvr_colsum': (_i, [_vp, _vp, _i, _i, _i64, _i, _vp, _sz, _vp]),
    'hvr_pack_conv_weight': (_i, [_vp, _vp, _vp, _i, _i, _i, _i, _i, _vp]),
    'hvr_pack_conv_weights_multi': (_i, [_vp, _i, _i64, _i, _vp]),
    'hvr_transpose_multi': (_i, [_vp, _i, _i, _vp]),
    'hvr_unpack_conv_wgrad': (_i, [_vp, _vp, _vp, _i, _i, _i, _i, _i, _vp]),
    'hvr_unpack_conv_wgrads_multi': (_i, [_vp, _i, _i64, _i, _vp]),
    'hvr_det_loss': (_i, [_vp, _i, _i, _i, _i, _vp, _vp, _vp, _vp, _i, _f, _f, _f, _vp, _vp, _vp]),
    'hvr_det_loss_sampled': (_i, [_vp, _i, _i, _i, _i, _vp, _vp, _vp, _vp, _i, _vp, _f, _vp, _vp, _vp]),
    'hvr_max_iou_assign_workspace_bytes': (_sz, [_i, _i]),
    'hvr_max_iou_assign': (_i, [_vp, _i, _i, _vp, _i, _vp, _f, _f, _f, _f, _vp, _vp, _vp, _sz, _vp]),
    'hvr_sample_pos_neg': (_i, [_vp, _vp, _i, _i, _i, _f, _vp, _vp, _vp]),
    'hvr_box_targets': (_i, [_vp, _i, _i, _vp, _vp, _vp, _vp, _vp, _i, _vp, _vp, _f, _i, _vp, _vp, _vp, _vp, _vp]),
    'hvr_rpn_loss': (_i, [_vp, _i, _i, _i, _vp, _vp, _vp, _vp, _vp, _f, _vp, _vp, _vp]),
    'hvr_ce_rows': (_i, [_vp, _i, _i, _i, _vp, _i, _vp, _vp]),
    'hvr_triplet_margin': (_i, [_vp, _i64, _vp, _i64, _i, _i, _i, _vp, _vp, _vp, _i, _f, _i, _vp, _sz, _vp, _vp, _vp, _vp]),
    'hvr_ingest_frame': (_i, [_vp, _i, _i, _i64, _vp, _i, _i, _i, _i, _vp, _vp, _i, _vp]),
    'hvr_ingest_frame_flip': (_i, [_vp, _i, _i, _i64, _vp, _i, _i, _i, _i, _vp, _vp, _i, _i, _vp]),
    'hvr_merge_aug_proposals_workspace_bytes': (_sz, [_i, _i, _i]),
    'hvr_merge_aug_proposals': (_i, [_vp, _vp, _i, _i, _i, _vp, _vp, _vp, _f, _i, _vp, _vp, _vp, _sz, _vp]),
    'hvr_map_aug_rois': (_i, [_vp, _i, _i, _i, _vp, _vp, _vp, _vp, _vp]),
    'hvr_merge_aug_dets': (_i, [_vp, _vp, _i, _i, _i, _vp, _vp, _vp, _vp, _vp, _vp]),
    'hvr_mining_argreduce': (_i, [_vp, _i, _i, _i64, _vp, _vp, _vp, _vp]),
    'hvr_roi_align_fwd': (_i, [_vp, _vp, _vp, _i, _i, _i, _i, _i, _i, _i, _f, _i, _i, _i, _vp]),
    'hvr_roi_align_bwd': (_i, [_vp, _vp, _vp, _i, _i, _i, _i, _i, _i, _i, _f, _i, _i, _vp]),
    'hvr_deform_im2col_supported': (_i, [_i, _i, _i]),
    'hvr_deform_im2col': (_i, [_vp, _vp, _vp, _i, _i, _i, _i, _i, _i, _i, _i, _i, _i, _i, _i64, _i, _vp]),
    'hvr_nms_workspace_bytes': (_sz, [_i]),
    'hvr_nms_first': (_i, [_vp, _i, _f, _i, _i, _vp, _vp, _vp, _sz, _vp]),
    'hvr_nms': (_i, [_vp, _i, _f, _i, _vp, _vp, _vp, _sz, _vp]),
    'hvr_rpn_workspace_bytes': (_sz, [_i, _i, _i, _i, _i]),
    'hvr_rpn_proposals': (_i, [ctypes.POINTER(RpnDesc), _vp, _sz, _vp]),
    'hvr_rpn_wide_frames': (_i, [_i]),
    'hvr_det_decode': (_i, [_vp, _i, _i, _i, _i, _vp, _i, _vp, _vp, _f, _f, _f, _f, _vp, _vp, _vp]),
    'hvr_multiclass_nms_workspace_bytes': (_sz, [_i, _i]),
    'hvr_multiclass_nms': (_i, [_vp, _vp, _i, _i, _f, _f, _i, _vp, _vp, _vp, _vp, _sz, _vp]),
    'hvr_soft_nms_workspace_bytes': (_sz, [_i]),
    'hvr_soft_nms': (_i, [_vp, _i, _f, _i, _f, _f, _vp, _vp, _vp, _vp, _sz, _vp]),
    'hvr_multiclass_soft_nms_workspace_bytes': (_sz, [_i, _i, _i]),
    'hvr_multiclass_soft_nms': (_i, [_vp, _vp, _i, _i, _i, _f, _f, _i, _f, _f, _i, _vp, _vp, _vp, _vp, _sz, _vp]),
    'hvr_seq_nms_workspace_bytes': (_sz, [_i, _i, _i]),
    'hvr_seq_nms': (_i, [_vp, _vp, _i, _i, _i, _f, _f, _f, _i, _i, _vp, _vp, _vp, _vp, _sz, _vp]),
    'hvr_seq_nms_phases': (_i, [_vp, _vp, _i, _i, _i, _f, _f, _f, _i, _i, _vp, _vp, _vp, _vp, _sz, _i, _vp]),
    'hvr_seq_nms_batched_workspace_bytes': (_sz, [_i, _i, _i, _i, _i]),
    'hvr_seq_nms_batched': (_i, [_vp, _vp, _i, _vp, _i, _i, _i, _f, _f, _f, _i, _i, _vp, _vp, _vp, _vp, _vp, _vp, _vp, _i, _vp, _sz, _vp]),
    'hvr_cast': (_i, [_vp, _vp, _i64, _i, _i, _vp]),
    'hvr_cast_scaled': (_i, [_vp, _vp, _i64, _i, _i, _f, _vp]),
    'hvr_permute_nchw_nhwc': (_i, [_vp, _vp, _i, _i, _i, _i, _i, _i, _vp]),
    'hvr_transpose_pad': (_i, [_vp, _vp, _i, _i, _i64, _i64, _i, _vp]),
}

_lib = None


def build(force=False):
    script = os.path.join(_HERE, 'csrc', 'build.sh')
    if force and os.path.exists(LIB_PATH):
        os.remove(LIB_PATH)
        for f in os.listdir(os.path.join(_HERE, 'csrc', 'build')) if os.path.isdir(os.path.join(_HERE, 'csrc', 'build')) else []:
            os.remove(os.path.join(_HERE, 'csrc', 'build', f))
    subprocess.run(['bash', script], check=True)
    return LIB_PATH


def lib():
    global _lib
    if _lib is None:
        if not os.path.exists(LIB_PATH):
            raise HvrError('libhvr_hip.so is missing: run `python -c "import __graft_entry__ as g; g.build()"` '
                           '(there is no CPU or PyTorch fallback for the HVR hot path)')
        handle = ctypes.CDLL(LIB_PATH)
        for name, (res, args) in SYMBOLS.items():
            fn = getattr(handle, name)
            fn.restype = res
            fn.argtypes = args
        if handle.hvr_abi_version() != ABI_VERSION:
            raise HvrError('libhvr_hip.so has ABI version %d, this binding needs %d: rebuild it (hvrnet_amd/csrc/build.sh)'
                           % (handle.hvr_abi_version(), ABI_VERSION))
        _lib = handle
    return _lib


def _check(rc, what):
    if rc != 0:
        raise HvrError('%s failed (%d): %s' % (what, rc, lib().hvr_last_error().decode()))


def _raw_stream(device=None):
    idx = torch._C._cuda_getDevice() if device is None or device.index is None else device.index
    return torch._C._cuda_getCurrentRawStream(idx)


def _stream():
    return ctypes.c_void_p(_raw_stream())


def _dt(t):
    if t.dtype == torch.float32:
        return HVR_F32
    if t.dtype == torch.bfloat16:
        return HVR_BF16
    if t.dtype == torch.float16:
        return HVR_F16
    if t.dtype == SPLIT:
        return HVR_F16S
    raise HvrError('unsupported tensor dtype %s (float32 / bfloat16 / float16 / the split-half container int32)' % t.dtype)


def _need_cuda(*ts):
    for t in ts:
        if t is not None and not t.is_cuda:
            raise NotImplementedError('hvr_hip ops run on the GPU only; got a %s tensor' % t.device)


def _ptr(t):
    return ctypes.c_void_p(t.data_ptr()) if t is not None else None


_prof = None


class _Span(object):
    __slots__ = ('tag', 'work', 'start')

    def __init__(self, tag, work):
        self.tag, self.work = tag, work

    def __enter__(self):
        self.start = torch.cuda.Event(enable_timing=True)
        self.start.record(torch.cuda.current_stream())

    def __exit__(self, *exc):
        end = torch.cuda.Event(enable_timing=True)
        end.record(torch.cuda.current_stream())
        _prof['spans'].append((self.tag, self.work, self.start, end))


class _NoSpan(object):
    def __enter__(self):
        return None

    def __exit__(self, *exc):
        return False


_NOSPAN = _NoSpan()


def _span(tag, work=0.0):
    if _prof is None or (tag.split(' ')[0] not in _prof['tags'] and '*' not in _prof['tags']):
        return _NOSPAN
    return _Span(tag, work)


def profile_begin(tags=('*',), detail=False):
    global _prof
    _prof = dict(tags=set(tags), spans=[], detail=detail)


def profile_end(raw=False):
    global _prof
    spans, _prof = _prof['spans'], None
    torch.cuda.synchronize()
    if raw:
        return [(tag, work, s.elapsed_time(e)) for tag, work, s, e in spans]
    out = {}
    for tag, work, s, e in spans:
        d = out.setdefault(tag, dict(calls=0, ms=0.0, work=0.0))
        d['calls'] += 1
        d['ms'] += s.elapsed_time(e)
        d['work'] += work
    return out


_zero_pages = {}


def zero_page(device):
    z = _zero_pages.get(device)
    if z is None:
        z = torch.zeros(256, dtype=torch.uint8, device=device)
        torch.cuda.current_stream(device).synchronize()
        _zero_pages[device] = z
    return z


def kstep(dtype):
    return 32 if dtype == torch.float32 else 64


SPLIT_WEIGHT_SCALE = 64.0
SPLIT_ACT_SCALE = 16.0


def _split_factors(out_is_f32, alpha):
    if alpha is not None:
        return float(alpha), 1.0
    if out_is_f32:
        return 1.0 / (SPLIT_WEIGHT_SCALE * SPLIT_ACT_SCALE), 1.0
    return 1.0 / SPLIT_WEIGHT_SCALE, SPLIT_ACT_SCALE


def as_operand(t, dtype):
    t = t.contiguous()
    if dtype == SPLIT:
        return cast(t.float(), SPLIT, scale=SPLIT_WEIGHT_SCALE)
    return t.to(dtype)


def gemm(a, w, bias=None, resid=None, relu=False, out_f32=False, out=None, staging=None, tile=None, alpha=None):
    _need_cuda(a, w, bias, resid)
    assert a.dim() == 2 and w.dim() == 2 and a.shape[1] == w.shape[1], (a.shape, w.shape)
    assert a.stride(1) == 1 and w.stride(1) == 1
    M, K = a.shape
    N = w.shape[0]
    if out is None:
        out = torch.empty((M, N), dtype=torch.float32 if out_f32 else a.dtype, device=a.device)
    d = GemmDesc(A=a.data_ptr(), B=w.data_ptr(), C=out.data_ptr(), M=M, N=N, K=K,
                 lda=a.stride(0), ldb=w.stride(0), ldc=out.stride(0),
                 bias=bias.data_ptr() if bias is not None else None,
                 resid=resid.data_ptr() if resid is not None else None,
                 ldr=resid.stride(0) if resid is not None else 0,
                 relu=int(relu), out_f32=int(out.dtype == torch.float32 and a.dtype != torch.float32),
                 dtype=_dt(a), staging=STAGING if staging is None else staging,
                 tile_hint=TILE_HINT if tile is None else tile)
    if a.dtype == SPLIT:
        if resid is not None and out.dtype == torch.float32:
            raise HvrError('split-half gemm: a residual cannot be combined with an f32 output (the residual carries the activation scale)')
        d.alpha, d.beta = _split_factors(out.dtype == torch.float32, alpha)
    nbytes = lib().hvr_gemm_fewrow_workspace_bytes(ctypes.byref(d)) if _fewrow[0] else 0
    if nbytes:
        ws = _workspace(nbytes, a.device, 'gemm_fewrow')
        d.ws, d.ws_bytes = ws.data_ptr(), ws.numel()
    with _span('gemm' if not (_prof and _prof['detail']) else 'gemm M%d N%d K%d' % (M, N, K), 2.0 * M * N * K):
        _check(lib().hvr_gemm(ctypes.byref(d), _stream()), 'hvr_gemm')
    return out


def gemm_splitk(a, w, staging=None, tile=None, out=None):
    _need_cuda(a, w)
    assert a.dim() == 2 and w.dim() == 2 and a.shape[1] == w.shape[1] and a.dtype == w.dtype, (a.shape, w.shape)
    assert a.stride(1) == 1 and w.stride(1) == 1
    M, K = a.shape
    N = w.shape[0]
    if out is None:
        out = torch.empty((M, N), dtype=torch.float32, device=a.device)
    else:
        assert out.dtype == torch.float32 and tuple(out.shape) == (M, N) and out.is_contiguous() and out.device == a.device
    d = GemmDesc(A=a.data_ptr(), B=w.data_ptr(), C=out.data_ptr(), M=M, N=N, K=K, lda=a.stride(0), ldb=w.stride(0), ldc=N,
                 bias=None, resid=None, ldr=0, relu=0, out_f32=int(a.dtype != torch.float32), dtype=_dt(a),
                 staging=STAGING if staging is None else staging, tile_hint=TILE_HINT if tile is None else tile)
    nbytes = lib().hvr_gemm_splitk_workspace_bytes(M, N, K, _dt(a))
    ws = _workspace(nbytes, a.device, 'splitk') if nbytes else None
    with _span('gemm' if not (_prof and _prof['detail']) else 'gemm M%d N%d K%d splitk' % (M, N, K), 2.0 * M * N * K):
        _check(lib().hvr_gemm_splitk(ctypes.byref(d), _ptr(ws), nbytes, _stream()), 'hvr_gemm_splitk')
    return out


def gemm_splitk_batched(a, w, out=None):
    _need_cuda(a, w)
    assert a.dim() == 3 and w.dim() == 3 and a.shape[0] == w.shape[0] and a.shape[2] == w.shape[2] and a.dtype == w.dtype
    assert a.stride(2) == 1 and w.stride(2) == 1 and a.stride(1) == a.shape[2] and w.stride(1) == w.shape[2]
    G, M, K = a.shape
    N = w.shape[1]
    if out is None:
        out = torch.empty((G, M, N), dtype=torch.float32, device=a.device)
    d = GemmDesc(A=a.data_ptr(), B=w.data_ptr(), C=out.data_ptr(), M=M, N=N, K=K, lda=K, ldb=K, ldc=N, bias=None, resid=None, ldr=0, relu=0,
                 out_f32=int(a.dtype != torch.float32), dtype=_dt(a), staging=STAGING, tile_hint=TILE_HINT)
    nbytes = lib().hvr_gemm_splitk_batched_workspace_bytes(M, N, K, _dt(a), G)
    ws = _workspace(nbytes, a.device, 'splitk_batched') if nbytes else None
    with _span('gemm' if not (_prof and _prof['detail']) else 'gemm %dx M%d N%d K%d splitk batched' % (G, M, N, K), 2.0 * G * M * N * K):
        _check(lib().hvr_gemm_splitk_batched(ctypes.byref(d), G, a.stride(0), w.stride(0), M * N, _ptr(ws), nbytes, _stream()), 'hvr_gemm_splitk_batched')
    return out


def conv2d_nhwc(x, w, bias=None, resid=None, relu=False, stride=1, pad=0, dil=1, out_f32=False, staging=None, tile=None, out=None, alpha=None):
    _need_cuda(x, w, bias, resid)
    B, H, W, Cin = x.shape
    Cout, KH, KW, _ = w.shape
    OH = (H + 2 * pad - dil * (KH - 1) - 1) // stride + 1
    OW = (W + 2 * pad - dil * (KW - 1) - 1) // stride + 1
    odt = torch.float32 if out_f32 else x.dtype
    if out is not None:
        assert tuple(out.shape) == (B, OH, OW, Cout) and out.dtype == odt and out.is_contiguous() and out.device == x.device, \
            (tuple(out.shape), (B, OH, OW, Cout), out.dtype)
        y = out
    else:
        y = torch.empty((B, OH, OW, Cout), dtype=odt, device=x.device)
    d = ConvDesc(x=x.data_ptr(), w=w.data_ptr(), y=y.data_ptr(), B=B, H=H, W=W, Cin=Cin, Cout=Cout, KH=KH, KW=KW,
                 stride=stride, pad=pad, dil=dil,
                 bias=bias.data_ptr() if bias is not None else None,
                 resid=resid.data_ptr() if resid is not None else None,
                 relu=int(relu), out_f32=int(out_f32 and x.dtype != torch.float32), dtype=_dt(x),
                 staging=STAGING if staging is None else staging, tile_hint=TILE_HINT if tile is None else tile,
                 zero=zero_page(x.device).data_ptr())
    if x.dtype == SPLIT:
        if resid is not None and out_f32:
            raise HvrError('split-half conv: a residual cannot be combined with an f32 output (the residual carries the activation scale)')
        d.alpha, d.beta = _split_factors(bool(out_f32), alpha)
    nbytes = lib().hvr_conv2d_splitk_workspace_bytes(ctypes.byref(d)) if _fewrow[0] else 0
    if nbytes:
        ws = _workspace(nbytes, x.device, 'conv_splitk')
        d.ws, d.ws_bytes = ws.data_ptr(), ws.numel()
    tag, work = 'conv', 2.0 * B * OH * OW * Cout * KH * KW * Cin
    if _prof is not None and ('*' in _prof['tags'] or 'conv' in _prof['tags'] or 'conv_expand' in _prof['tags']):
        if lib().hvr_conv2d_path(ctypes.byref(d)) == 1:
            tag, work = 'conv_expand', float((B * OH * OW * (Cin + (2 if resid is not None else 1) * Cout) + Cout * Cin) * x.element_size())
        if _prof['detail']:
            tag = '%s %dx%d %d->%d k%d s%d d%d%s' % (tag, H, W, Cin, Cout, KH, stride, dil, '+res' if resid is not None else '')
    with _span(tag, work):
        _check(lib().hvr_conv2d_nhwc(ctypes.byref(d), _stream()), 'hvr_conv2d_nhwc')
    return y


def _tail_desc(h, x, w, bias, stride2, relu, y):
    B, OH, OW, C1 = h.shape
    _, H2, W2, C2 = x.shape
    return TailDesc(h=h.data_ptr(), x=x.data_ptr(), w=w.data_ptr(), y=y.data_ptr() if y is not None else 1 << 20, B=B, OH=OH, OW=OW, C1=C1,
                    H2=H2, W2=W2, C2=C2, stride2=int(stride2), Cout=w.shape[0], bias=bias.data_ptr(), relu=int(relu), dtype=_dt(h))


def bottleneck_tail_supported(h, x, w, bias, stride2):
    if not (h.is_cuda and h.dtype in (torch.bfloat16, torch.float16) and x.dtype == h.dtype and h.is_contiguous() and x.is_contiguous()):
        return False
    return bool(lib().hvr_bottleneck_tail_supported(ctypes.byref(_tail_desc(h, x, w, bias, stride2, True, None))))


def bottleneck_tail(h, x, w, bias, stride2=1, relu=True, out=None):
    _need_cuda(h, x, w, bias)
    B, OH, OW, C1 = h.shape
    Cout = w.shape[0]
    if out is not None:
        assert tuple(out.shape) == (B, OH, OW, Cout) and out.dtype == h.dtype and out.is_contiguous()
        y = out
    else:
        y = torch.empty((B, OH, OW, Cout), dtype=h.dtype, device=h.device)
    d = _tail_desc(h, x, w, bias, stride2, relu, y)
    tag, work = 'conv_expand', float((h.numel() + B * OH * OW * x.shape[3] + y.numel() + w.numel()) * h.element_size())
    if _prof is not None and _prof['detail']:
        tag = 'conv_expand tail %dx%d %d+%d->%d s%d' % (OH, OW, C1, x.shape[3], Cout, stride2)
    with _span(tag, work):
        _check(lib().hvr_bottleneck_tail(ctypes.byref(d), _stream()), 'hvr_bottleneck_tail')
    return y


def _tail_next_desc(h, x, resid, w, bias, stride2, wn, bias_n, y, hn):
    B, OH, OW, C1 = h.shape
    ph = 1 << 20
    if x is not None:
        t = _tail_desc(h, x, w, bias, stride2, True, y)
    else:
        t = TailDesc(h=h.data_ptr(), x=None, w=w.data_ptr(), y=y.data_ptr() if y is not None else ph, B=B, OH=OH, OW=OW, C1=C1,
                     H2=OH, W2=OW, C2=0, stride2=1, Cout=w.shape[0], bias=bias.data_ptr(), relu=1, dtype=_dt(h))
    d = TailNextDesc(tail=t, resid=resid.data_ptr() if resid is not None else None, wn=wn.data_ptr(), bias_n=bias_n.data_ptr(),
                     hn=hn.data_ptr() if hn is not None else ph, Cn=wn.shape[0])
    if h.dtype == SPLIT:
        d.alpha, d.beta = _split_factors(False, None)
    return d


def bottleneck_tail_next_supported(h, x, resid, w, bias, stride2, wn, bias_n):
    ts = [t for t in (h, x, resid) if t is not None]
    if not all(t.is_cuda and t.dtype in (torch.bfloat16, torch.float16, SPLIT) and t.dtype == h.dtype and t.is_contiguous() for t in ts):
        return False
    if h.dtype == SPLIT and (x is not None or wn.dtype != SPLIT or w.dtype != SPLIT):
        return False
    if (x is None) == (resid is None) or wn.dim() != 2 or wn.shape[1] != w.shape[0] or not wn.is_contiguous():
        return False
    return bool(lib().hvr_bottleneck_tail_next_supported(ctypes.byref(_tail_next_desc(h, x, resid, w, bias, stride2, wn, bias_n, None, None))))


def bottleneck_tail_next(h, x, resid, w, bias, wn, bias_n, stride2=1, out=None):
    _need_cuda(h, w, bias, wn, bias_n)
    B, OH, OW, C1 = h.shape
    Cout, Cn = w.shape[0], wn.shape[0]
    if out is not None:
        assert tuple(out.shape) == (B, OH, OW, Cout) and out.dtype == h.dtype and out.is_contiguous()
        y = out
    else:
        y = torch.empty((B, OH, OW, Cout), dtype=h.dtype, device=h.device)
    hn = torch.empty((B, OH, OW, Cn), dtype=h.dtype, device=h.device)
    d = _tail_next_desc(h, x, resid, w, bias, stride2, wn, bias_n, y, hn)
    side = x if x is not None else resid
    tag = 'conv_expand'
    work = float((h.numel() + B * OH * OW * side.shape[3] + y.numel() + hn.numel() + w.numel() + wn.numel()) * h.element_size())
    if _prof is not None and _prof['detail']:
        tag = 'conv_expand tail+next %dx%d %d+%d->%d->%d' % (OH, OW, C1, x.shape[3] if x is not None else 0, Cout, Cn)
    with _span(tag, work):
        _check(lib().hvr_bottleneck_tail_next(ctypes.byref(d), _stream()), 'hvr_bottleneck_tail_next')
    return y, hn


def _close_sampled_desc(h, w, bias, resid, stride, relu, y):
    B, OH, OW, C1 = h.shape
    _, RH, RW, Cout = resid.shape
    d = CloseSampledDesc(h=h.data_ptr(), w=w.data_ptr(), resid=resid.data_ptr(), y=y.data_ptr() if y is not None else 1 << 20, B=B, OH=OH, OW=OW,
                         C1=C1, Cout=Cout, RH=RH, RW=RW, rstride=int(stride), bias=bias.data_ptr(), relu=int(relu), dtype=_dt(h))
    if h.dtype == SPLIT:
        d.alpha, d.beta = _split_factors(False, None)
    return d


def bottleneck_close_sampled_supported(h, w, bias, resid, stride):
    if not (h.is_cuda and h.dtype in (torch.bfloat16, torch.float16, SPLIT) and resid.dtype == h.dtype and w.dtype == h.dtype
            and h.is_contiguous() and resid.is_contiguous() and w.is_contiguous() and h.dim() == 4 and resid.dim() == 4):
        return False
    if h.shape[0] != resid.shape[0] or w.numel() != resid.shape[3] * h.shape[3] or w.shape[0] != resid.shape[3]:
        return False
    return bool(lib().hvr_bottleneck_close_sampled_supported(ctypes.byref(_close_sampled_desc(h, w, bias, resid, stride, True, None))))


def bottleneck_close_sampled(h, w, bias, resid, stride=2, relu=True, out=None):
    _need_cuda(h, w, bias, resid)
    B, OH, OW, C1 = h.shape
    _, RH, RW, Cout = resid.shape
    assert h.is_contiguous() and resid.is_contiguous() and w.is_contiguous() and resid.dtype == h.dtype and w.dtype == h.dtype
    assert w.shape[0] == Cout and w.numel() == Cout * C1 and resid.shape[0] == B, (tuple(w.shape), tuple(resid.shape))
    if out is not None:
        assert tuple(out.shape) == (B, OH, OW, Cout) and out.dtype == h.dtype and out.is_contiguous()
        y = out
    else:
        y = torch.empty((B, OH, OW, Cout), dtype=h.dtype, device=h.device)
    d = _close_sampled_desc(h, w, bias, resid, stride, relu, y)
    tag, work = 'conv_expand', float((B * OH * OW * (C1 + 2 * Cout) + Cout * C1) * h.element_size())
    if _prof is not None and _prof['detail']:
        tag = 'conv_expand sampled %dx%d<-%dx%d %d->%d k1+res s%d' % (OH, OW, RH, RW, C1, Cout, stride)
    with _span(tag, work):
        _check(lib().hvr_bottleneck_close_sampled(ctypes.byref(d), _stream()), 'hvr_bottleneck_close_sampled')
    return y


def conv2d_path(B, H, W, Cin, Cout, k=1, stride=1, pad=0, dil=1, dtype=torch.bfloat16, resid=True, bias=True, out_f32=False, tile=0):
    fake = 1 << 20
    d = ConvDesc(x=fake, w=fake, y=fake, B=B, H=H, W=W, Cin=Cin, Cout=Cout, KH=k, KW=k, stride=stride, pad=pad, dil=dil,
                 bias=fake if bias else None, resid=fake if resid else None, relu=1, out_f32=int(out_f32),
                 dtype={torch.bfloat16: HVR_BF16, torch.float16: HVR_F16, SPLIT: HVR_F16S}.get(dtype, HVR_F32), staging=STAGING,
                 tile_hint=tile, zero=fake)
    return int(lib().hvr_conv2d_path(ctypes.byref(d)))


def im2col_stem(img, dtype, kp=192):
    _need_cuda(img)
    assert img.dtype == torch.float32 and img.is_contiguous()
    B, _, H, W = img.shape
    OH, OW = (H + 6 - 7) // 2 + 1, (W + 6 - 7) // 2 + 1
    cols = torch.empty((B * OH * OW, kp), dtype=torch.float32 if dtype == SPLIT else dtype, device=img.device)
    _check(lib().hvr_im2col_stem(_ptr(img), _ptr(cols), B, H, W, kp, _dt(cols), _stream()), 'hvr_im2col_stem')
    return (cast(cols, SPLIT) if dtype == SPLIT else cols), OH, OW


def stem_fused(img, wpk, bias):
    _need_cuda(img, wpk, bias)
    assert img.dtype == torch.float32 and img.is_contiguous() and wpk.dtype in (torch.bfloat16, torch.float16)
    split = wpk.dim() == 4
    assert tuple(wpk.shape) == ((2, 64, 7, 32) if split else (64, 7, 32)) and (not split or wpk.dtype == torch.float16) and wpk.is_contiguous()
    B, _, H, W = img.shape
    CH, CW = (H + 6 - 7) // 2 + 1, (W + 6 - 7) // 2 + 1
    PH, PW = (CH + 2 - 3) // 2 + 1, (CW + 2 - 3) // 2 + 1
    out = torch.empty((B, PH, PW, 64), dtype=SPLIT if split else wpk.dtype, device=img.device)
    with _span('stem', 2.0 * B * CH * CW * 64 * 147):
        _check(lib().hvr_stem_fused_dtype(_ptr(img), _ptr(wpk), _ptr(bias), _ptr(out), B, H, W, HVR_F16S if split else _dt(wpk), _stream()),
               'hvr_stem_fused')
    return out


def stem_split_weights(wf):
    wf = wf * (SPLIT_WEIGHT_SCALE * SPLIT_ACT_SCALE)
    hi = wf.half()
    lo = (wf - hi.float()).half()
    return torch.stack([hi, lo], 0).contiguous()


def stem_split_bias(b):
    return (b * SPLIT_ACT_SCALE).contiguous()


def maxpool3x3s2_nhwc(x):
    _need_cuda(x)
    if x.dtype == SPLIT:
        return cast(maxpool3x3s2_nhwc(cast(x, torch.float32)), SPLIT)
    B, H, W, C = x.shape
    OH, OW = (H + 2 - 3) // 2 + 1, (W + 2 - 3) // 2 + 1
    y = torch.empty((B, OH, OW, C), dtype=x.dtype, device=x.device)
    _check(lib().hvr_maxpool3x3s2_nhwc(_ptr(x), _ptr(y), B, H, W, C, _dt(x), _stream()), 'hvr_maxpool3x3s2_nhwc')
    return y


_ws_cache = {}


_fewrow = [False]


def fewrow_enabled():
    return _fewrow[0]


@contextlib.contextmanager
def fewrow_split(on=True):
    prev = _fewrow[0]
    _fewrow[0] = bool(on)
    try:
        yield
    finally:
        _fewrow[0] = prev


BIG_TILE_HINT = 16
TWO_LEVEL_HINT = 18


@contextlib.contextmanager
def throughput_mode(on=True):
    global TILE_HINT
    prev = TILE_HINT
    if on and TILE_HINT == 0:
        TILE_HINT = BIG_TILE_HINT
    try:
        yield
    finally:
        TILE_HINT = prev


_hip_rt = [None]
_masked_streams = {}


def cu_masked_stream(device, first_cu, n_cus, total_cus=256):
    dev = torch.device(device)
    key = (dev.index if dev.index is not None else torch.cuda.current_device(), int(first_cu), int(n_cus))
    if key in _masked_streams:
        return _masked_streams[key][1]
    if _hip_rt[0] is None:
        rt = ctypes.CDLL('libamdhip64.so')
        rt.hipExtStreamCreateWithCUMask.argtypes = [ctypes.POINTER(ctypes.c_void_p), ctypes.c_uint32, ctypes.POINTER(ctypes.c_uint32)]
        rt.hipExtStreamCreateWithCUMask.restype = ctypes.c_int
        _hip_rt[0] = rt
    if not (0 <= first_cu and n_cus > 0 and first_cu + n_cus <= total_cus):
        raise HvrError('CU mask [%d, %d) outside [0, %d)' % (first_cu, first_cu + n_cus, total_cus))
    words = (total_cus + 31) // 32
    mask = (ctypes.c_uint32 * words)()
    for cu in range(first_cu, first_cu + n_cus):
        mask[cu // 32] |= 1 << (cu % 32)
    handle = ctypes.c_void_p()
    with torch.cuda.device(key[0]):
        rc = _hip_rt[0].hipExtStreamCreateWithCUMask(ctypes.byref(handle), words, mask)
    if rc != 0:
        raise HvrError('hipExtStreamCreateWithCUMask failed (%d)' % rc)
    st = torch.cuda.ExternalStream(handle.value, device=torch.device('cuda', key[0]))
    _masked_streams[key] = (handle, st)
    return st


_ws_captured = set()
_ws_retired = []


def _workspace(nbytes, device, tag):
    key = (tag, device.index if isinstance(device, torch.device) else str(device), _raw_stream(device if isinstance(device, torch.device) else None))
    ws = _ws_cache.get(key)
    capturing = torch.cuda.is_current_stream_capturing()
    if ws is None or ws.numel() < nbytes:
        if capturing:
            raise HvrError('scratch buffer %r must grow (%d -> %d bytes) inside a stream capture: warm the largest shapes up first'
                           % (tag, 0 if ws is None else ws.numel(), nbytes))
        if ws is not None and key in _ws_captured:
            _ws_retired.append(ws)
            _ws_captured.discard(key)
        ws = torch.empty(int(nbytes), dtype=torch.uint8, device=device)
        _ws_cache[key] = ws
    if capturing:
        _ws_captured.add(key)
    return ws


def relation_fwd(q, k, v, scale, staging=None):
    _need_cuda(q, k, v)
    Mq, D = q.shape
    Mk = k.shape[0]
    assert k.shape[1] == D and v.shape == (Mk, D) and q.dtype == k.dtype == v.dtype
    o = torch.empty((Mq, D), dtype=q.dtype, device=q.device)
    nbytes = lib().hvr_relation_workspace_bytes(Mq, Mk, D, _dt(q))
    ws = _workspace(nbytes, q.device, 'relation')
    if q.dtype == SPLIT:
        scale = float(scale) / (SPLIT_ACT_SCALE * SPLIT_ACT_SCALE)
    with _span('relation_full' if Mq == Mk else 'relation_key', 4.0 * Mq * Mk * D):
        _check(lib().hvr_relation_fwd(_ptr(q), q.stride(0), _ptr(k), k.stride(0), _ptr(v), v.stride(0), _ptr(o), o.stride(0),
                                      Mq, Mk, D, float(scale), _dt(q), STAGING if staging is None else staging,
                                      _ptr(ws), ws.numel(), _stream()), 'hvr_relation_fwd')
    return o


def relation_fwd_grouped(q, k, v, scale, groups, staging=None, exact=False):
    _need_cuda(q, k, v)
    G = int(groups)
    assert G >= 1 and q.shape[0] % G == 0 and k.shape[0] % G == 0
    Mq, Mk, D = q.shape[0] // G, k.shape[0] // G, q.shape[1]
    assert k.shape[1] == D and v.shape == k.shape and q.dtype == k.dtype == v.dtype
    if G == 1:
        return relation_fwd(q, k, v, scale, staging)
    o = torch.empty((G * Mq, D), dtype=q.dtype, device=q.device)
    nbytes = lib().hvr_relation_grouped_workspace_bytes(G, Mq, Mk, D, _dt(q))
    ws = _workspace(nbytes, q.device, 'relation_grouped')
    if q.dtype == SPLIT:
        scale = float(scale) / (SPLIT_ACT_SCALE * SPLIT_ACT_SCALE)
    with _span('relation_full' if Mq == Mk else 'relation_key', 4.0 * G * Mq * Mk * D):
        _check(lib().hvr_relation_fwd_grouped(_ptr(q), q.stride(0), Mq * q.stride(0), _ptr(k), k.stride(0), Mk * k.stride(0),
                                              _ptr(v), v.stride(0), Mk * v.stride(0), _ptr(o), o.stride(0), Mq * o.stride(0), G,
                                              Mq, Mk, D, float(scale), _dt(q), STAGING if staging is None else staging, int(bool(exact)),
                                              _ptr(ws), ws.numel(), _stream()), 'hvr_relation_fwd_grouped')
    return o


def relation_ldp(Mk):
    return (Mk + 127) // 128 * 128


def relation_probs(q, k, scale, staging=None, out=None):
    _need_cuda(q, k)
    Mq, D = q.shape
    Mk = k.shape[0]
    ldp = relation_ldp(Mk)
    if out is None:
        P = torch.empty((Mq, ldp), dtype=q.dtype, device=q.device)
    else:
        assert out.shape == (Mq, ldp) and out.dtype == q.dtype and out.device == q.device and out.is_contiguous()
        P = out
    ws = _workspace(lib().hvr_relation_probs_workspace_bytes(Mq, Mk), q.device, 'relation_probs')
    _check(lib().hvr_relation_probs(_ptr(q), q.stride(0), _ptr(k), k.stride(0), _ptr(P), ldp, Mq, Mk, D, float(scale), _dt(q),
                                    STAGING if staging is None else staging, _ptr(ws), ws.numel(), _stream()), 'hvr_relation_probs')
    return P


def relation_dscore(P, dP, dO, O, scale):
    _need_cuda(P, dP, dO, O)
    assert P.shape == dP.shape and P.is_contiguous() and dP.is_contiguous() and dO.stride(1) == 1 and O.stride(1) == 1
    dS = torch.empty_like(P)
    _check(lib().hvr_relation_dscore(_ptr(P), _ptr(dP), _ptr(dO), dO.stride(0), _ptr(O), O.stride(0), _ptr(dS), P.shape[0],
                                     P.shape[1], dO.shape[1], float(scale), _dt(P), _stream()), 'hvr_relation_dscore')
    return dS


def im2col_nhwc(x, KH, KW, pad, dil):
    _need_cuda(x)
    x = x.contiguous()
    B, H, W, Cin = x.shape
    OH, OW = H + 2 * pad - dil * (KH - 1), W + 2 * pad - dil * (KW - 1)
    cols = torch.empty((B * OH * OW, KH * KW * Cin), dtype=x.dtype, device=x.device)
    _check(lib().hvr_im2col_nhwc(_ptr(x), _ptr(cols), B, H, W, Cin, KH, KW, pad, dil, _dt(x), _stream()), 'hvr_im2col_nhwc')
    return cols


def scale_rows(w, scale):
    _need_cuda(w, scale)
    w = w.contiguous()
    out = torch.empty_like(w)
    R = w.shape[0]
    _check(lib().hvr_scale_rows(_ptr(w), _ptr(scale.float().contiguous()), _ptr(out), R, w.numel() // R, _dt(w), _stream()), 'hvr_scale_rows')
    return out


def sgd_step(param_flat, grad_flat, momentum_buf, lr, momentum, weight_decay, grad_scale=1.0, max_norm=0.0, first_step=False):
    _need_cuda(param_flat, grad_flat, momentum_buf)
    assert param_flat.dtype == grad_flat.dtype == momentum_buf.dtype == torch.float32
    assert param_flat.is_contiguous() and grad_flat.is_contiguous() and momentum_buf.is_contiguous()
    assert param_flat.numel() == grad_flat.numel() == momentum_buf.numel()
    ws = _workspace(lib().hvr_sgd_workspace_bytes(), param_flat.device, 'sgd')
    _check(lib().hvr_sgd_step(_ptr(param_flat), _ptr(grad_flat), _ptr(momentum_buf), param_flat.numel(), float(lr), float(momentum),
                              float(weight_decay), float(grad_scale), float(max_norm), _ptr(ws), ws.numel(), int(first_step),
                              _stream()), 'hvr_sgd_step')


def relu_bwd(dy, y):
    _need_cuda(dy, y)
    dy, y = dy.contiguous(), y.contiguous()
    assert dy.shape == y.shape and dy.dtype == y.dtype and dy.numel() % 4 == 0
    dz = torch.empty_like(dy)
    _check(lib().hvr_relu_bwd(_ptr(dy), _ptr(y), _ptr(dz), dy.numel(), _dt(dy), _stream()), 'hvr_relu_bwd')
    return dz


def relu_bwd_t(dy, y, ldt, dzt_out=None):
    _need_cuda(dy, y)
    dy, y = dy.contiguous(), y.contiguous()
    assert dy.dim() == 2 and dy.shape == y.shape and dy.dtype == y.dtype
    R, C = dy.shape
    dz = torch.empty_like(dy)
    if dzt_out is None:
        dzt = torch.empty((C, ldt), dtype=dy.dtype, device=dy.device)
    else:
        assert tuple(dzt_out.shape) == (C, ldt) and dzt_out.dtype == dy.dtype and dzt_out.is_contiguous()
        dzt = dzt_out
    _check(lib().hvr_relu_bwd_t(_ptr(dy), _ptr(y), _ptr(dz), _ptr(dzt), ldt, R, C, _dt(dy), _stream()), 'hvr_relu_bwd_t')
    return dz, dzt


def im2col_t(x, KH, KW, pad, dil, ldt, out=None):
    _need_cuda(x)
    x = x.contiguous()
    B, H, W, Cin = x.shape
    if out is None:
        out = torch.empty((KH * KW * Cin, ldt), dtype=x.dtype, device=x.device)
    else:
        assert tuple(out.shape) == (KH * KW * Cin, ldt) and out.dtype == x.dtype and out.is_contiguous()
    _check(lib().hvr_im2col_t(_ptr(x), _ptr(out), ldt, B, H, W, Cin, KH, KW, pad, dil, _dt(x), _stream()), 'hvr_im2col_t')
    return out


def colsum(dy, out=None):
    _need_cuda(dy)
    assert dy.dim() == 2 and dy.stride(1) == 1
    if out is None:
        db = torch.empty(dy.shape[1], dtype=torch.float32, device=dy.device)
    else:
        assert out.dtype == torch.float32 and tuple(out.shape) == (dy.shape[1],) and out.is_contiguous() and out.device == dy.device
        db = out
    nbytes = lib().hvr_colsum_workspace_bytes(dy.shape[0], dy.shape[1])
    ws = _workspace(nbytes, dy.device, 'colsum') if nbytes else None
    _check(lib().hvr_colsum(_ptr(dy), _ptr(db), dy.shape[0], dy.shape[1], dy.stride(0), _dt(dy), _ptr(ws), nbytes, _stream()), 'hvr_colsum')
    return db


def pack_conv_weight(w, scale, dtype):
    _need_cuda(w, scale)
    assert w.dtype == torch.float32 and w.is_contiguous() and scale.dtype == torch.float32 and scale.is_contiguous()
    Cout, Cin, KH, KW = w.shape
    out = torch.empty((Cout, KH, KW, Cin), dtype=dtype, device=w.device)
    _check(lib().hvr_pack_conv_weight(_ptr(w), _ptr(scale), _ptr(out), Cout, Cin, KH, KW, _dt(out), _stream()), 'hvr_pack_conv_weight')
    return out


class PackItem(ctypes.Structure):
    _fields_ = [('w', ctypes.c_void_p), ('scale', ctypes.c_void_p), ('out', ctypes.c_void_p), ('first', ctypes.c_int64),
                ('Cout', ctypes.c_int32), ('Cin', ctypes.c_int32), ('KK', ctypes.c_int32), ('pad_', ctypes.c_int32)]


class TransposeItem(ctypes.Structure):
    _fields_ = [('src', ctypes.c_void_p), ('dst', ctypes.c_void_p), ('lds', ctypes.c_int64), ('ldd', ctypes.c_int64),
                ('R', ctypes.c_int32), ('C', ctypes.c_int32), ('first_tile', ctypes.c_int32), ('tiles_c', ctypes.c_int32),
                ('dcols', ctypes.c_int32), ('pad_', ctypes.c_int32)]


def items_to_device(items, device):
    arr = (type(items[0]) * len(items))(*items)
    host = torch.frombuffer(bytearray(bytes(arr)), dtype=torch.uint8)
    return host.to(device)


def pack_conv_weights_multi(items_dev, n, total, dtype):
    code = {torch.bfloat16: HVR_BF16, torch.float16: HVR_F16}[dtype]
    _check(lib().hvr_pack_conv_weights_multi(_ptr(items_dev), n, total, code, _stream()), 'hvr_pack_conv_weights_multi')


def transpose_multi(items_dev, n, tiles):
    _check(lib().hvr_transpose_multi(_ptr(items_dev), n, tiles, _stream()), 'hvr_transpose_multi')


def unpack_conv_wgrads_multi(items_dev, n, total, accumulate=True):
    _check(lib().hvr_unpack_conv_wgrads_multi(_ptr(items_dev), n, total, int(accumulate), _stream()), 'hvr_unpack_conv_wgrads_multi')


def unpack_conv_wgrad(dw, scale, shape, accumulate_into=None):
    _need_cuda(dw, scale)
    Cout, Cin, KH, KW = shape
    assert dw.dtype == torch.float32 and dw.is_contiguous() and dw.numel() == Cout * Cin * KH * KW
    if accumulate_into is not None:
        out = accumulate_into
        assert out.dtype == torch.float32 and out.is_contiguous() and tuple(out.shape) == tuple(shape)
    else:
        out = torch.empty(shape, dtype=torch.float32, device=dw.device)
    _check(lib().hvr_unpack_conv_wgrad(_ptr(dw), _ptr(scale), _ptr(out), Cout, Cin, KH, KW, int(accumulate_into is not None), _stream()),
           'hvr_unpack_conv_wgrad')
    return out


def _loss_operands(labels, label_weights, bbox_targets, bbox_weights, n):
    assert labels.numel() == label_weights.numel() == n, 'labels / label_weights: one value per anchor (rows * A) or row'
    assert bbox_targets.numel() == bbox_weights.numel() == 4 * n, 'bbox_targets / bbox_weights: four values per anchor or row'
    return labels.contiguous(), label_weights.float().contiguous(), bbox_targets.float().contiguous(), bbox_weights.float().contiguous()


def det_loss(logits, cls_off, reg_off, ncls, labels, label_weights, bbox_targets, bbox_weights, beta=1.0, w_cls=1.0, w_bbox=1.0):
    _need_cuda(logits, labels, label_weights, bbox_targets, bbox_weights)
    assert logits.dtype == torch.float32 and logits.is_contiguous() and labels.dtype == torch.long
    labels, lw, bt, bw = _loss_operands(labels, label_weights, bbox_targets, bbox_weights, logits.shape[0])
    out3 = torch.empty(3, dtype=torch.float32, device=logits.device)
    dlogits = torch.empty_like(logits)
    _check(lib().hvr_det_loss(_ptr(logits), logits.shape[1], cls_off, reg_off, ncls, _ptr(labels), _ptr(lw), _ptr(bt), _ptr(bw),
                              logits.shape[0], float(beta), float(w_cls), float(w_bbox), _ptr(out3), _ptr(dlogits), _stream()),
           'hvr_det_loss')
    return out3, dlogits



def max_iou_assign(boxes, gts, pos_iou_thr, neg_iou_thr, min_pos_iou, valid=None):
    _need_cuda(boxes, gts, valid)
    assert boxes.dtype == torch.float32 and boxes.dim() == 2 and boxes.stride(1) == 1 and boxes.shape[1] >= 4
    gts = gts.contiguous().float()
    n, k = boxes.shape[0], gts.shape[0]
    if n == 0 or k == 0:
        raise ValueError('No gt or bboxes')
    lo, hi = (0.0, float(neg_iou_thr)) if isinstance(neg_iou_thr, (int, float)) else (float(neg_iou_thr[0]), float(neg_iou_thr[1]))
    if valid is not None:
        valid = valid.contiguous().view(torch.uint8) if valid.dtype == torch.bool else valid.contiguous()
        assert valid.dtype == torch.uint8 and valid.numel() == n
    gt_inds = torch.empty(n, dtype=torch.long, device=boxes.device)
    max_ov = torch.empty(n, dtype=torch.float32, device=boxes.device)
    nbytes = lib().hvr_max_iou_assign_workspace_bytes(n, k)
    ws = _workspace(nbytes, boxes.device, 'assign')
    _check(lib().hvr_max_iou_assign(_ptr(boxes), boxes.stride(0), n, _ptr(gts), k, _ptr(valid), float(pos_iou_thr), lo, hi,
                                    float(min_pos_iou), _ptr(gt_inds), _ptr(max_ov), _ptr(ws), nbytes, _stream()), 'hvr_max_iou_assign')
# ... 524 lines not shown
```

### include/hvr_hip.h

```cpp
#ifndef HVR_HIP_H_
#define HVR_HIP_H_

#include <stddef.h>
#include <stdint.h>

#ifdef __cplusplus
extern "C" {
#endif

#define HVR_OK 0
#define HVR_EINVAL (-1)
#define HVR_EUNSUPPORTED (-2)
#define HVR_ELAUNCH (-3)
#define HVR_EWORKSPACE (-4)

#define HVR_F32 0
#define HVR_BF16 1
#define HVR_F16 2
#define HVR_F16S 3

#define HVR_LAYOUT_NCHW 0
#define HVR_LAYOUT_NHWC 1

int hvr_abi_version(void);
const char* hvr_last_error(void);

typedef struct hvr_gemm_desc {
  const void* A; const void* B; void* C;
  int32_t M, N, K;
  int64_t lda, ldb, ldc;
  const float* bias;
  const void* resid;
  int64_t ldr;
  int32_t relu;
  int32_t out_f32;
  int32_t dtype;
  int32_t staging;
  int32_t tile_hint;
  void* ws; size_t ws_bytes;
  float alpha;
  float beta;
} hvr_gemm_desc;
size_t hvr_gemm_fewrow_workspace_bytes(const hvr_gemm_desc* d);
int hvr_gemm(const hvr_gemm_desc* d, void* stream);
size_t hvr_gemm_splitk_workspace_bytes(int M, int N, int K, int dtype);
int hvr_gemm_splitk(const hvr_gemm_desc* d, void* ws, size_t ws_bytes, void* stream);
size_t hvr_gemm_splitk_batched_workspace_bytes(int M, int N, int K, int dtype, int count);
int hvr_gemm_splitk_batched(const hvr_gemm_desc* d, int count, int64_t stride_a, int64_t stride_b, int64_t stride_c, void* ws, size_t ws_bytes,
                            void* stream);

typedef struct hvr_conv_desc {
  const void* x; const void* w; void* y;
  int32_t B, H, W, Cin, Cout, KH, KW, stride, pad, dil;
  const float* bias;
  const void* resid;
  int32_t relu, out_f32, dtype, staging, tile_hint;
  const void* zero;
  void* ws; size_t ws_bytes;
  float alpha, beta;
} hvr_conv_desc;
int hvr_conv2d_nhwc(const hvr_conv_desc* d, void* stream);
size_t hvr_conv2d_splitk_workspace_bytes(const hvr_conv_desc* d);
int hvr_conv2d_path(const hvr_conv_desc* d);

typedef struct hvr_tail_desc {
  const void* h; const void* x; const void* w; void* y;
  int32_t B, OH, OW, C1, H2, W2, C2, stride2, Cout;
  const float* bias;
  int32_t relu, dtype;
} hvr_tail_desc;
int hvr_bottleneck_tail(const hvr_tail_desc* d, void* stream);
int hvr_bottleneck_tail_supported(const hvr_tail_desc* d);

typedef struct hvr_tail_next_desc {
  hvr_tail_desc tail;
  const void* resid;
  const void* wn; const float* bias_n; void* hn;
  int32_t Cn;
  float alpha, beta;
} hvr_tail_next_desc;
int hvr_bottleneck_tail_next(const hvr_tail_next_desc* d, void* stream);
int hvr_bottleneck_tail_next_supported(const hvr_tail_next_desc* d);

typedef struct hvr_close_sampled_desc {
  const void* h; const void* w; const void* resid; void* y;
  int32_t B, OH, OW, C1, Cout, RH, RW, rstride;
  const float* bias;
  int32_t relu, dtype;
  float alpha, beta;
} hvr_close_sampled_desc;
int hvr_bottleneck_close_sampled(const hvr_close_sampled_desc* d, void* stream);
int hvr_bottleneck_close_sampled_supported(const hvr_close_sampled_desc* d);

int hvr_im2col_stem(const float* img, void* cols, int B, int H, int W, int KP, int dtype, void* stream);
int hvr_stem_fused(const float* img, const void* wpk, const float* bias, void* out, int B, int H, int W, void* stream);
int hvr_stem_fused_dtype(const float* img, const void* wpk, const float* bias, void* out, int B, int H, int W, int dtype, void* stream);
int hvr_maxpool3x3s2_nhwc(const void* x, void* y, int B, int H, int W, int C, int dtype, void* stream);

size_t hvr_relation_workspace_bytes(int Mq, int Mk, int D, int dtype);
int hvr_relation_fwd(const void* Q, int64_t ldq, const void* K, int64_t ldk, const void* V, int64_t ldv,
                     void* O, int64_t ldo, int Mq, int Mk, int D, float scale, int dtype, int staging,
                     void* ws, size_t ws_bytes, void* stream);

size_t hvr_relation_grouped_workspace_bytes(int groups, int Mq, int Mk, int D, int dtype);
int hvr_relation_fwd_grouped(const void* Q, int64_t ldq, int64_t gsq, const void* K, int64_t ldk, int64_t gsk,
                             const void* V, int64_t ldv, int64_t gsv, void* O, int64_t ldo, int64_t gso, int groups,
                             int Mq, int Mk, int D, float scale, int dtype, int staging, int exact, void* ws, size_t ws_bytes, void* stream);

size_t hvr_relation_probs_workspace_bytes(int Mq, int Mk);
int hvr_relation_probs(const void* Q, int64_t ldq, const void* K, int64_t ldk, void* P, int64_t ldp, int Mq, int Mk, int D,
                       float scale, int dtype, int staging, void* ws, size_t ws_bytes, void* stream);
int hvr_relation_dscore(const void* P, const void* dP, const void* dO, int64_t ldgo, const void* O, int64_t ldo, void* dS,
                        int Mq, int64_t ldp, int D, float scale, int dtype, void* stream);

int hvr_relu_bwd(const void* dY, const void* Y, void* dZ, int64_t n, int dtype, void* stream);
size_t hvr_colsum_workspace_bytes(int M, int N);
int hvr_colsum(const void* dY, float* db, int M, int N, int64_t ld, int dtype, void* ws, size_t ws_bytes, void* stream);
int hvr_det_loss(const float* logits, int ldl, int cls_off, int reg_off, int ncls, const int64_t* labels, const float* label_weights,
                 const float* bbox_targets, const float* bbox_weights, int R, float beta, float w_cls, float w_bbox, float* out3,
                 float* dlogits, void* stream);

int hvr_im2col_nhwc(const void* x, void* cols, int B, int H, int W, int Cin, int KH, int KW, int pad, int dil, int dtype, void* stream);
int hvr_im2col_t(const void* x, void* colsT, int64_t ldt, int B, int H, int W, int Cin, int KH, int KW, int pad, int dil, int dtype, void* stream);
int hvr_relu_bwd_t(const void* dY, const void* Y, void* dZ, void* dZt, int64_t ldt, int R, int C, int dtype, void* stream);
int hvr_scale_rows(const void* w, const float* scale, void* out, int R, int64_t C, int dtype, void* stream);
int hvr_pack_conv_weight(const float* w, const float* scale, void* out, int Cout, int Cin, int KH, int KW, int out_dtype, void* stream);
int hvr_unpack_conv_wgrad(const float* dw, const float* scale, float* out, int Cout, int Cin, int KH, int KW, int accumulate, void* stream);
typedef struct { const float* w; const float* scale; void* out; int64_t first; int32_t Cout, Cin, KK, pad_; } hvr_pack_item;
typedef struct { const void* src; void* dst; int64_t lds, ldd; int32_t R, C, first_tile, tiles_c, dcols, pad_; } hvr_transpose_item;
int hvr_pack_conv_weights_multi(const hvr_pack_item* items_dev, int n, int64_t total, int out_dtype, void* stream);
typedef struct { float* out; const float* scale; const float* dw; int64_t first; int32_t Cout, Cin, KK, pad_; } hvr_unpack_item;
int hvr_unpack_conv_wgrads_multi(const hvr_unpack_item* items_dev, int n, int64_t total, int accumulate, void* stream);
int hvr_transpose_multi(const hvr_transpose_item* items_dev, int n, int tiles, void* stream);

size_t hvr_sgd_workspace_bytes(void);
int hvr_sgd_step(float* param, const float* grad, float* momentum_buf, int64_t n, float lr, float momentum, float weight_decay,
                 float grad_scale, float max_norm, float* ws, size_t ws_bytes, int first_step, void* stream);

int hvr_roi_align_fwd(const void* feat, const float* rois, void* out, int B, int C, int H, int W, int K,
                      int PH, int PW, float spatial_scale, int sample_num, int dtype, int layout, void* stream);
int hvr_roi_align_bwd(const float* grad_out, const float* rois, float* grad_feat, int B, int C, int H, int W,
                      int K, int PH, int PW, float spatial_scale, int sample_num, int layout, void* stream);

int hvr_deform_im2col_supported(int Cin, int deformable_groups, int dtype);
int hvr_deform_im2col(const void* x, const float* om, void* col, int B, int H, int W, int Cin, int KH, int KW, int stride, int pad,
                      int dil, int deformable_groups, int modulated, int64_t ldo, int dtype, void* stream);

size_t hvr_nms_workspace_bytes(int n);
int hvr_nms(const float* dets, int n, float thr, int ge_semantics, int64_t* keep, int32_t* n_keep,
            void* ws, size_t ws_bytes, void* stream);
int hvr_nms_first(const float* dets, int n, float thr, int ge_semantics, int max_keep, int64_t* keep, int32_t* n_keep,
                  void* ws, size_t ws_bytes, void* stream);

typedef struct hvr_rpn_desc {
  const float* cls; const float* reg;
  int32_t T, H, W, A, anchor_stride;
  const float* base_anchors; const float* means; const float* stds;
  float img_h, img_w, wh_ratio_clip;
  int32_t nms_pre, nms_post, max_num;
  float nms_thr;
  float* proposals; int32_t* counts;
  int32_t cls_pitch, reg_pitch;
} hvr_rpn_desc;
size_t hvr_rpn_workspace_bytes(int T, int H, int W, int A, int nms_pre);
int hvr_rpn_proposals(const hvr_rpn_desc* d, void* ws, size_t ws_bytes, void* stream);
int hvr_rpn_wide_frames(int frames);

int hvr_det_decode(const float* logits, int ldl, int cls_off, int reg_off, int ncls, const float* rois, int R,
                   const float* means, const float* stds, float wh_ratio_clip, float img_h, float img_w,
                   float scale_factor, float* scores, float* boxes, void* stream);
size_t hvr_multiclass_nms_workspace_bytes(int R, int ncls);
int hvr_multiclass_nms(const float* boxes, const float* scores, int R, int ncls, float score_thr, float iou_thr,
                       int max_num, float* dets, int64_t* labels, int32_t* n_out, void* ws, size_t ws_bytes,
                       void* stream);

size_t hvr_soft_nms_workspace_bytes(int n);
int hvr_soft_nms(const float* dets, int n, float iou_thr, int method, float sigma, float min_score, float* out_dets, int64_t* inds,
                 int32_t* n_out, void* ws, size_t ws_bytes, void* stream);
size_t hvr_multiclass_soft_nms_workspace_bytes(int P, int R, int ncls);
int hvr_multiclass_soft_nms(const float* boxes, const float* scores, int P, int R, int ncls, float score_thr, float iou_thr, int method,
                            float sigma, float min_score, int max_num, float* dets, int64_t* labels, int32_t* n_out, void* ws,
                            size_t ws_bytes, void* stream);

size_t hvr_seq_nms_workspace_bytes(int F, int R, int ncls);
int hvr_seq_nms(const float* boxes, const float* scores, int F, int R, int ncls, float score_thr, float link_thr, float nms_thr,
                int rescore, int max_num, float* dets, int64_t* labels, int32_t* n_out, void* ws, size_t ws_bytes, void* stream);
int hvr_seq_nms_phases(const float* boxes, const float* scores, int F, int R, int ncls, float score_thr, float link_thr, float nms_thr,
                       int rescore, int max_num, float* dets, int64_t* labels, int32_t* n_out, void* ws, size_t ws_bytes, int phases,
                       void* stream);
size_t hvr_seq_nms_batched_workspace_bytes(int P, int Ftot, int R, int ncls, int tubes);
int hvr_seq_nms_batched(const float* boxes, const float* scores, int P, const int32_t* frame_start, int Ftot, int R, int ncls, float score_thr,
                        float link_thr, float nms_thr, int rescore, int max_num, float* dets, int64_t* labels, int32_t* n_out,
                        int32_t* tube_ids, int32_t* tubes, float* tube_scores, int32_t* tube_start, int max_tubes, void* ws, size_t ws_bytes,
                        void* stream);

int hvr_cast(const void* in, void* out, int64_t n, int from_dtype, int to_dtype, void* stream);
int hvr_cast_scaled(const void* in, void* out, int64_t n, int from_dtype, int to_dtype, float scale, void* stream);
int hvr_permute_nchw_nhwc(const void* in, void* out, int B, int C, int HW, int to_nhwc, int from_dtype,
                          int to_dtype, void* stream);
int hvr_transpose_pad(const void* in, void* out, int R, int C, int64_t ldx, int64_t ldt, int dtype, void* stream);

size_t hvr_max_iou_assign_workspace_bytes(int n, int k);
int hvr_max_iou_assign(const float* boxes, int ldb, int n, const float* gts, int k, const uint8_t* valid, float pos_iou_thr,
                       float neg_iou_lo, float neg_iou_hi, float min_pos_iou, int64_t* gt_inds, float* max_overlaps, void* ws,
                       size_t ws_bytes, void* stream);
int hvr_sample_pos_neg(const int64_t* cls, const float* keys, int n, int num, int num_expected_pos, float neg_pos_ub, int64_t* inds,
                       int32_t* counts, void* stream);
int hvr_box_targets(const float* boxes, int ldb, int n, const float* gts, const int64_t* gt_labels, const int64_t* gt_inds,
                    const int64_t* inds, const int32_t* counts, int num, const float* means4, const float* stds4, float pos_weight,
                    int scatter, int64_t* labels, float* label_weights, float* bbox_targets, float* bbox_weights, void* stream);
int hvr_rpn_loss(const float* o, int ldo, int A, int rows, const int64_t* labels, const float* label_weights, const float* bbox_targets,
                 const float* bbox_weights, const int32_t* counts, float beta, float* out2, float* d_o, void* stream);
int hvr_ce_rows(const float* logits, int ldl, int cls_off, int ncls, const int64_t* labels, int R, float* loss, void* stream);
int hvr_triplet_margin(const void* q, int64_t ldq, const void* k, int64_t ldk, int D, int Mq, int Mk, const int64_t* anchor_idx,
                       const int64_t* pos_idx, const int64_t* neg_idx, int n, float margin, int dtype, float* ws, size_t ws_bytes,
                       float* out2, float* dq, float* dk, void* stream);
int hvr_mining_argreduce(const float* aff, int Mq, int Mk, int64_t ld, const int64_t* labels, const int64_t* all_labels, int64_t* out4,
                         void* stream);
int hvr_det_loss_sampled(const float* logits, int ldl, int cls_off, int reg_off, int ncls, const int64_t* labels,
                         const float* label_weights, const float* bbox_targets, const float* bbox_weights, int R,
                         const int32_t* sel_counts, float beta, float* out3, float* dlogits, void* stream);

int hvr_ingest_frame(const uint8_t* src, int src_h, int src_w, int64_t src_pitch, float* dst, int new_h, int new_w, int pad_h, int pad_w,
                     const float* mean3, const float* std3, int to_rgb, void* stream);
int hvr_ingest_frame_flip(const uint8_t* src, int src_h, int src_w, int64_t src_pitch, float* dst, int new_h, int new_w, int pad_h, int pad_w,
                          const float* mean3, const float* std3, int to_rgb, int flip, void* stream);

size_t hvr_merge_aug_proposals_workspace_bytes(int A, int T, int mx);
int hvr_merge_aug_proposals(const float* proposals, const int32_t* counts, int A, int T, int mx, const float* img_w,
                            const float* scale_factor, const int32_t* flip, float nms_thr, int max_num, float* merged,
                            int32_t* merged_counts, void* ws, size_t ws_bytes, void* stream);
int hvr_map_aug_rois(const float* merged, int A, int T, int max_num, const float* img_w, const float* scale_factor, const int32_t* flip,
                     float* rois, void* stream);
int hvr_merge_aug_dets(const float* boxes, const float* scores, int A, int R, int ncls, const float* img_w, const float* scale_factor,
                       const int32_t* flip, float* merged_boxes, float* merged_scores, void* stream);

#ifdef __cplusplus
}
#endif
#endif
```

Before: 177.7 frames/s.

## Add four-slot half-K ring pipeline to big-tile GEMM for multi-tap convs

Adds a RING variant of the big-tile kernel. It splits each 64-element K step into two 32-element halves stored as 64-byte rows with a new swizzle, and keeps four LDS slots in flight. Waits become partial vmcnt counts instead of a full drain at the end of each K step. The variant is routed by default for bf16/f16 convs with KH*KW>1 and N==256. The change also specializes the epilogue on whether a residual exists, and sets the persistent grid to the device CU count instead of a fixed 256. Risks are more DMA instructions per K step, a changed LDS bank-conflict pattern, and waitcnt accounting errors.

After: 174.5 frames/s. 1.8% lower.

```diff
diff --git a/hvrnet_amd/csrc/bigtile.hip b/hvrnet_amd/csrc/bigtile.hip
--- a/hvrnet_amd/csrc/bigtile.hip
+++ b/hvrnet_amd/csrc/bigtile.hip
@@ -8,7 +8,7 @@
 namespace {
 
 constexpr int BG_BN = 256, BG_NT = 512, BG_WN = 4, BG_FN = 4, BG_WCOLS = BG_FN * 16;
-constexpr int BG_B_SLOTS = BG_BN * 8 / BG_NT;
+__host__ __device__ constexpr int bg_ring_key(int row) { return ((((row >> 2) ^ (row >> 3)) & 1) << 1) | ((row >> 3) & 1); }
 
 __device__ __forceinline__ uint32_t bg_lds_off(const void* p) {
   return (uint32_t)(uintptr_t)(const __attribute__((address_space(3))) char*)p;
@@ -35,15 +35,20 @@
 
 }
 
-template <typename T, int FM0, int FM1>
+template <typename T, int FM0, int FM1, bool RING = false>
 __global__ __launch_bounds__(BG_NT) void big_tile_kernel(const GemmParams p) {
   constexpr bool SPLIT = std::is_same<T, f16s_t>::value;
+  static_assert(!(RING && SPLIT), "split half keeps the two-stage loop (six phases per K-step)");
   constexpr int EB = (int)sizeof(T), KSG = 128;
   constexpr int BKE = SPLIT ? 32 : 64;
   constexpr int BM = (FM0 + FM1) * 16;
-  constexpr int A_BYTES = BM * 128, STAGE = A_BYTES + BG_BN * 128;
-  constexpr int A_SLOTS = (BM * 8 + BG_NT - 1) / BG_NT;
-  constexpr int LAST_WAVES = (BM * 8 - (A_SLOTS - 1) * BG_NT) / 64;
+  constexpr int ROWB = RING ? 64 : 128;
+  constexpr int RPP = BG_NT * 16 / ROWB;
+  constexpr int FRAG = 16 * ROWB;
+  constexpr int A_BYTES = BM * ROWB, STAGE = A_BYTES + BG_BN * ROWB;
+  constexpr int A_SLOTS = (BM + RPP - 1) / RPP, B_SLOTS = BG_BN / RPP;
+  constexpr int LAST_WAVES = (BM - (A_SLOTS - 1) * RPP) * (ROWB / 16) / 64;
+  static_assert(LAST_WAVES <= BG_WN, "the partial A slot belongs to waves of group 0");
   extern __shared__ __attribute__((aligned(16))) char smem[];
   const int tid = threadIdx.x, lane = tid & 63;
   const int wave = __builtin_amdgcn_readfirstlane(tid >> 6);
@@ -61,7 +66,8 @@
   dbg_t[0] = wall_clock64();
 #endif
 
-  const int l_row = tid >> 3, l_chunk = ((tid & 7) ^ (l_row & 7)) * 16;
+  const int l_row = RING ? tid >> 2 : tid >> 3;
+  const int l_chunk = RING ? ((tid & 3) ^ bg_ring_key(l_row)) * 16 : ((tid & 7) ^ (l_row & 7)) * 16;
   int a_bias = 0;
   if (p.conv) a_bias = (int)(((long)p.pad * p.W + p.pad) * p.Cin * EB);
   const char* const rs_a = (const char*)p.A - a_bias;
@@ -74,7 +80,7 @@
   const int cRowB = is_conv ? p.W * p.Cin * EB : 0, cPixB = is_conv ? p.Cin * EB : 0;
 
   constexpr bool SEG2 = !SPLIT;
-  struct TileState { int a_off[A_SLOTS], a_off2[SEG2 ? A_SLOTS : 1], b_off[BG_B_SLOTS]; unsigned oob[A_SLOTS]; int m0, n0; };
+  struct TileState { int a_off[A_SLOTS], a_off2[SEG2 ? A_SLOTS : 1], b_off[B_SLOTS]; unsigned oob[A_SLOTS]; int m0, n0; };
   auto setup = [&](int tile, TileState& st) {
     const __attribute__((address_space(4))) GemmParams* kq =
         (const __attribute__((address_space(4))) GemmParams*)__builtin_amdgcn_kernarg_segment_ptr();
@@ -85,7 +91,7 @@
     int a_yx[A_SLOTS];
 #pragma unroll
     for (int i = 0; i < A_SLOTS; ++i) {
-      int m = st.m0 + i * 64 + l_row;
+      int m = st.m0 + i * RPP + l_row;
       m = m < kq->M ? m : kq->M - 1;
       if constexpr (SEG2) st.a_off2[i] = 0;
       if (kq->conv || (SEG2 && kq->s2 > 0)) {
@@ -105,7 +111,7 @@
       }
     }
 #pragma unroll
-    for (int i = 0; i < BG_B_SLOTS; ++i) st.b_off[i] = (int)((long)(st.n0 + i * 64 + l_row) * kq->ldb * EB) + l_chunk;
+    for (int i = 0; i < B_SLOTS; ++i) st.b_off[i] = (int)((long)(st.n0 + i * RPP + l_row) * kq->ldb * EB) + l_chunk;
 #pragma unroll
     for (int i = 0; i < A_SLOTS; ++i) st.oob[i] = 0u;
     if (kq->conv != 0) {
@@ -146,29 +152,37 @@
     const int keep = rst ? 0 : -1;
     kt_load &= keep; b_koff &= keep; t_cin0 &= keep; t_kx &= keep; t_ky &= keep; t_tap &= keep; a_koff &= keep;
   };
-  auto dma_a = [&](auto I, char* stage, bool nx) {
-    constexpr int i = decltype(I)::value;
-    if (i < A_SLOTS - 1 || wave < LAST_WAVES) {
+  auto dma_a = [&](auto I, char* stage, bool nx, auto KADD, auto CHK) {
+    constexpr int i = decltype(I)::value, kadd = decltype(KADD)::value;
+    if (!decltype(CHK)::value || i < A_SLOTS - 1 || wave < LAST_WAVES) {
       const unsigned ao = (unsigned)(nx ? ns.a_off[i] : cs.a_off[i]), ob = nx ? ns.oob[i] : cs.oob[i];
       const unsigned voff = ao | ((ob >> (t_tap & 31)) << 31);
       if constexpr (SEG2) {
         const bool s2 = kt_load >= k1_steps;
         const char* const base = s2 ? rs_a2 : rs_a;
         const unsigned vo = s2 ? (unsigned)(nx ? ns.a_off2[i] : cs.a_off2[i]) : voff;
-        const int so = s2 ? (kt_load - k1_steps) * KSG : a_koff;
+        const int so = (s2 ? (kt_load - k1_steps) * KSG : a_koff) + kadd;
         bg_load_lds16(base, stage + (i * BG_NT + wave * 64) * 16, vo, __builtin_amdgcn_readfirstlane(so));
       } else {
-        bg_load_lds16(rs_a, stage + (i * BG_NT + wave * 64) * 16, voff, __builtin_amdgcn_readfirstlane(a_koff));
+        bg_load_lds16(rs_a, stage + (i * BG_NT + wave * 64) * 16, voff, __builtin_amdgcn_readfirstlane(a_koff + kadd));
       }
     }
   };
-  auto dma_b = [&](auto I, char* stage, bool nx) {
-    constexpr int i = decltype(I)::value;
-    bg_load_lds16(rs_b, stage + A_BYTES + (i * BG_NT + wave * 64) * 16, (unsigned)(nx ? ns.b_off[i] : cs.b_off[i]), __builtin_amdgcn_readfirstlane(b_koff));
+  auto dma_b = [&](auto I, char* stage, bool nx, auto KADD) {
+    constexpr int i = decltype(I)::value, kadd = decltype(KADD)::value;
+    bg_load_lds16(rs_b, stage + A_BYTES + (i * BG_NT + wave * 64) * 16, (unsigned)(nx ? ns.b_off[i] : cs.b_off[i]), __builtin_amdgcn_readfirstlane(b_koff + kadd));
   };
-
-  static_for<A_SLOTS>([&](auto I) { dma_a(I, smem, false); });
-  static_for<BG_B_SLOTS>([&](auto I) { dma_b(I, smem, false); });
+  constexpr std::integral_constant<int, 0> K0{};
+  constexpr std::integral_constant<int, 64> K64{};
+  constexpr std::true_type CHECKED{};
+  constexpr std::false_type UNCHECKED{};
+
+  static_for<A_SLOTS>([&](auto I) { dma_a(I, smem, false, K0, CHECKED); });
+  static_for<B_SLOTS>([&](auto I) { dma_b(I, smem, false, K0); });
+  if constexpr (RING) {
+    static_for<A_SLOTS>([&](auto I) { dma_a(I, smem + STAGE, false, K64, CHECKED); });
+    static_for<B_SLOTS>([&](auto I) { dma_b(I, smem + STAGE, false, K64); });
+  }
 
   auto body = [&](auto FMC) {
   constexpr int FM = decltype(FMC)::value;
@@ -183,8 +197,9 @@
     for (int j = 0; j < BG_FN; ++j) acc[i][j] = f32x4{0.f, 0.f, 0.f, 0.f};
 
   const int frag_row = lane & 15, frag_grp = lane >> 4, swz = lane & 7;
-  const uint32_t a_lane = bg_lds_off(smem) + (wrow0 + frag_row) * 128 + ((frag_grp ^ swz) * 16);
-  const uint32_t b_lane = bg_lds_off(smem) + A_BYTES + (wn * BG_WCOLS + frag_row) * 128 + ((frag_grp ^ swz) * 16);
+  const int frag_pos = RING ? (frag_grp ^ bg_ring_key(frag_row)) * 16 : (frag_grp ^ swz) * 16;
+  const uint32_t a_lane = bg_lds_off(smem) + (wrow0 + frag_row) * ROWB + frag_pos;
+  const uint32_t b_lane = bg_lds_off(smem) + A_BYTES + (wn * BG_WCOLS + frag_row) * ROWB + frag_pos;
 
   const int nk = nk_real;
   if (round == 0) asm volatile("s_waitcnt vmcnt(0)" ::: "memory");
@@ -195,14 +210,16 @@
 
   {
     constexpr int G0 = (FM + 1) / 2;
-    constexpr int DMA_TOTAL = A_SLOTS + BG_B_SLOTS, DMA_FIRST = DMA_TOTAL / 2;
-    auto kloop = [&](auto WMC) __attribute__((always_inline)) {
+    constexpr int DMA_TOTAL = A_SLOTS + B_SLOTS, DMA_FIRST = DMA_TOTAL / 2;
+    auto kloop = [&](auto WMC, auto XC) __attribute__((always_inline)) {
     constexpr int wmc = decltype(WMC)::value;
     constexpr int dma_ph = wmc ? 0 : 1;
+    constexpr bool extra = decltype(XC)::value != 0;
+    constexpr int NPW = A_SLOTS - 1 + B_SLOTS + (extra ? 1 : 0);
     if constexpr (wmc != 0) __builtin_amdgcn_s_barrier();
     for (int kt = 0; kt < nk; ++kt) {
-      const uint32_t soff = (uint32_t)((kt + par) & 1) * STAGE;
-      char* nxt = smem + ((kt + 1 + par) & 1) * STAGE;
+      const uint32_t soff = (uint32_t)(RING ? (2 * kt + par) & 3 : (kt + par) & 1) * STAGE;
+      char* nxt = smem + (RING ? (2 * kt + 2 + par) & 3 : (kt + 1 + par) & 1) * STAGE;
       const uint32_t a0 = a_lane + soff, b0 = b_lane + soff;
       uint4 kb[BG_FN], qa[G0];
       const bool last = kt + 1 >= nk, pre = last && has_next;
@@ -211,29 +228,40 @@
       static_for<NPH>([&](auto PH) {
         constexpr int ph = decltype(PH)::value, term = ph >> 1, r0 = (ph & 1) ? G0 : 0, nr = (ph & 1) ? FM - G0 : G0;
         constexpr bool b_lo = term == 1, a_lo = SPLIT ? term == 2 : term == 1;
+        constexpr int HB = RING && b_lo ? STAGE : 0, HA = RING && a_lo ? STAGE : 0;
         if constexpr ((ph & 1) == 0)
-          static_for<BG_FN>([&](auto J) { kb[decltype(J)::value] = bg_read128<decltype(J)::value * 2048>(b_lo ? (b0 ^ 64u) : b0); });
+          static_for<BG_FN>([&](auto J) { kb[decltype(J)::value] = bg_read128<decltype(J)::value * FRAG + HB>(b_lo && !RING ? (b0 ^ 64u) : b0); });
         static_for<nr>([&](auto R) {
           constexpr int r = decltype(R)::value;
-          qa[r] = bg_read128<(r0 + r) * 2048>(a_lo ? (a0 ^ 64u) : a0);
+          qa[r] = bg_read128<(r0 + r) * FRAG + HA>(a_lo && !RING ? (a0 ^ 64u) : a0);
         });
         __builtin_amdgcn_sched_barrier(0);
-        if constexpr (ph < 3) {
+        if constexpr (RING) {
+          constexpr int half = ph >> 1;
+          constexpr std::integral_constant<int, half * 64> KH{};
+          char* const dst = nxt + half * STAGE;
+          if constexpr ((ph & 1) != 0) {
+            static_for<A_SLOTS - 1>([&](auto D) { dma_a(D, dst, pre, KH, UNCHECKED); });
+            static_for<B_SLOTS>([&](auto D) { dma_b(D, dst, pre, KH); });
+            if constexpr (extra) dma_a(std::integral_constant<int, A_SLOTS - 1>{}, dst, pre, KH, UNCHECKED);
+            if constexpr (wmc != 0) asm volatile("s_waitcnt vmcnt(%0)" :: "n"(NPW) : "memory");
+          }
+        } else if constexpr (ph < 3) {
           if constexpr (dma_ph == ph) {
             static_for<DMA_FIRST>([&](auto D) {
               constexpr int d = decltype(D)::value;
-              if constexpr (d < A_SLOTS) dma_a(std::integral_constant<int, d>{}, nxt, pre);
-              else dma_b(std::integral_constant<int, d - A_SLOTS>{}, nxt, pre);
+              if constexpr (d < A_SLOTS) dma_a(std::integral_constant<int, d>{}, nxt, pre, K0, CHECKED);
+              else dma_b(std::integral_constant<int, d - A_SLOTS>{}, nxt, pre, K0);
             });
           } else if constexpr (dma_ph + 1 == ph) {
             static_for<DMA_TOTAL - DMA_FIRST>([&](auto D) {
               constexpr int d = DMA_FIRST + decltype(D)::value;
-              if constexpr (d < A_SLOTS) dma_a(std::integral_constant<int, d>{}, nxt, pre);
-              else dma_b(std::integral_constant<int, d - A_SLOTS>{}, nxt, pre);
+              if constexpr (d < A_SLOTS) dma_a(std::integral_constant<int, d>{}, nxt, pre, K0, CHECKED);
+              else dma_b(std::integral_constant<int, d - A_SLOTS>{}, nxt, pre, K0);
             });
           }
         }
-        if constexpr (ph == NPH - 1) {
+        if constexpr (!RING && ph == NPH - 1) {
           if constexpr (wmc != 0) asm volatile("s_waitcnt vmcnt(0)" ::: "memory");
         }
         __builtin_amdgcn_sched_barrier(0);
@@ -247,7 +275,9 @@
         });
         __builtin_amdgcn_s_setprio(0);
         __builtin_amdgcn_sched_barrier(0);
-        if constexpr (ph == NPH - 1) {
+        if constexpr (RING) {
+          if constexpr ((ph & 1) != 0 && wmc == 0) asm volatile("s_waitcnt vmcnt(%0)" :: "n"(NPW) : "memory");
+        } else if constexpr (ph == NPH - 1) {
           if constexpr (wmc == 0) asm volatile("s_waitcnt vmcnt(0)" ::: "memory");
         }
         __builtin_amdgcn_s_barrier();
@@ -257,14 +287,22 @@
     };
     int wsel = wave;
     asm volatile("" : "+s"(wsel));
-    if (wsel >= BG_WN) kloop(std::integral_constant<int, 1>{});
-    else kloop(std::integral_constant<int, 0>{});
+    if (wsel >= BG_WN) {
+      kloop(std::integral_constant<int, 1>{}, std::integral_constant<int, 0>{});
+    } else {
+      if constexpr (RING) {
+        if (wsel < LAST_WAVES) kloop(std::integral_constant<int, 0>{}, std::integral_constant<int, 1>{});
+        else kloop(std::integral_constant<int, 0>{}, std::integral_constant<int, 0>{});
+      } else {
+        kloop(std::integral_constant<int, 0>{}, std::integral_constant<int, 0>{});
+      }
+    }
   }
 #ifdef HVR_DBG_BG_CLK
   if (round < 3) dbg_t[2 + 3 * round] = wall_clock64();
 #endif
 
-  char* const epi_base = smem + ((nk - 1 + par) & 1) * STAGE;
+  char* const epi_base = smem + (RING ? (2 * nk - 2 + par) & 3 : (nk - 1 + par) & 1) * STAGE;
   const __attribute__((address_space(4))) GemmParams* kp =
       (const __attribute__((address_space(4))) GemmParams*)__builtin_amdgcn_kernarg_segment_ptr();
   asm volatile("" : "+s"(kp));
@@ -354,6 +392,8 @@
     }
   } else
   {
+    auto epilogue = [&](auto RES) __attribute__((always_inline)) {
+    constexpr bool has_res = decltype(RES)::value;
     int etid = threadIdx.x;
     asm volatile("" : "+v"(etid));
     const int el = etid & 63, erow = el & 15, egrp = el >> 4;
@@ -372,7 +412,6 @@
       }
     }
     const int st_row = el >> 3, st_chunk = el & 7;
-    const bool has_res = kp->resid != nullptr;
     auto load_res = [&](int i, uint4 (&rv)[2]) {
 #pragma unroll
       for (int h = 0; h < 2; ++h) {
@@ -382,12 +421,12 @@
       }
     };
     uint4 rnext[2] = {make_uint4(0u, 0u, 0u, 0u), make_uint4(0u, 0u, 0u, 0u)};
-    if (has_res) load_res(0, rnext);
+    if constexpr (has_res) load_res(0, rnext);
     asm volatile("s_waitcnt lgkmcnt(0)" ::: "memory");
     __builtin_amdgcn_s_barrier();
 #pragma unroll
     for (int i = 0; i < FM; ++i) {
-      if (has_res) {
+      if constexpr (has_res) {
 #pragma unroll
         for (int h = 0; h < 2; ++h) {
           const uint4 v = h ? make_uint4(rnext[h].z, rnext[h].w, rnext[h].x, rnext[h].y) : rnext[h];
@@ -401,7 +440,7 @@
         float e[4];
 #pragma unroll
         for (int r = 0; r < 4; ++r) e[r] = acc[i][j][r] + bias[j][r];
-        if (has_res) {
+        if constexpr (has_res) {
           const uint2 rr = *reinterpret_cast<const uint2*>(slot);
           float r0_, r1_, r2_, r3_;
           unpack2<T>(rr.x, r0_, r1_);
@@ -422,17 +461,21 @@
         if (m < kp->M) *reinterpret_cast<uint4*>((unsigned short*)kp->C + (long)m * kp->ldc + n0 + wn * BG_WCOLS + st_chunk * 8) = v;
       }
     }
+    };
+    if (kp->resid != nullptr) epilogue(std::true_type{});
+    else epilogue(std::false_type{});
   }
 #ifdef HVR_DBG_BG_CLK
   if (round < 3) dbg_t[3 + 3 * round] = wall_clock64();
 #endif
   if (!has_next) break;
-  par = (par + nk) & 1;
+  par = RING ? (par + 2 * nk) & 3 : (par + nk) & 1;
   cs = ns;
   cur_tile = nxt_tile;
   nxt_tile = tile_of(round + 2);
   if (nxt_tile >= 0) setup(nxt_tile, ns);
   }
+  if constexpr (RING) asm volatile("s_waitcnt vmcnt(0)" ::: "memory");
 #ifdef HVR_DBG_BG_CLK
   asm volatile("s_waitcnt vmcnt(0)" ::: "memory");
   {
@@ -462,7 +505,9 @@
   if (p.N % BG_BN || p.K % bke || p.ldc % row_al || p.lda % row_al || p.ldb % row_al) return false;
   if (p.resid && (p.ldr % row_al || (reinterpret_cast<uintptr_t>(p.resid) & (split ? 127 : 15)))) return false;
   if (split && ((reinterpret_cast<uintptr_t>(p.A) | reinterpret_cast<uintptr_t>(p.B) | reinterpret_cast<uintptr_t>(p.C)) & 127)) return false;
-  if (p.tile_hint != kBigForce && (p.K < 256 || (p.resid && throughput && !split))) return false;
+  const bool forced = p.tile_hint == kBigForce || p.tile_hint == kBigRing;
+  if (split && p.tile_hint == kBigRing) return false;
+  if (!forced && (p.K < 256 || (p.resid && throughput && !split))) return false;
   if (p.conv && (p.Cin % bke || p.KH * p.KW > 32)) return false;
   const uintptr_t al = reinterpret_cast<uintptr_t>(p.A) | reinterpret_cast<uintptr_t>(p.B) | reinterpret_cast<uintptr_t>(p.C) |
                        reinterpret_cast<uintptr_t>(p.bias);
@@ -472,29 +517,55 @@
   static const int on = std::getenv("HVR_BIGTILE") ? std::atoi(std::getenv("HVR_BIGTILE")) : 1;
   constexpr int min_alone = 170;
   constexpr int min_shared = 96;
-  if (p.tile_hint == kBigForce) return true;
+  if (forced) return true;
   return on && tiles >= (throughput ? min_shared : min_alone) && tiles <= 4096;
 }
 
-template <typename T, int FM0, int FM1>
+static int device_cus() {
+  static std::atomic<int> cus[kMaxDevices];
+  int d = -1;
+  (void)hipGetDevice(&d);
+  const bool slot = d >= 0 && d < kMaxDevices;
+  int n = slot ? cus[d].load(std::memory_order_relaxed) : 0;
+  if (n > 0) return n;
+  if (d < 0 || hipDeviceGetAttribute(&n, hipDeviceAttributeMultiprocessorCount, d) != hipSuccess || n <= 0) n = 256;
+  if (slot) cus[d].store(n, std::memory_order_relaxed);
+  return n;
+}
+
+template <typename T, int FM0, int FM1, bool RING>
 static hipError_t launch_bigtile(const GemmParams& p, hipStream_t stream) {
   constexpr int BM = (FM0 + FM1) * 16, lds = 2 * (BM + BG_BN) * 128;
-  auto kern = big_tile_kernel<T, FM0, FM1>;
+  auto kern = big_tile_kernel<T, FM0, FM1, RING>;
   static std::atomic<unsigned> attr_set_dev{0};
   per_device_once(attr_set_dev, [&] {
     (void)hipFuncSetAttribute(reinterpret_cast<const void*>(kern), hipFuncAttributeMaxDynamicSharedMemorySize, lds);
   });
   const int tiles = ((p.M + BM - 1) / BM) * (p.N / BG_BN);
-  static const int nper = std::getenv("HVR_BIGTILE_WGS") ? std::atoi(std::getenv("HVR_BIGTILE_WGS")) : 256;
+  int nper = device_cus();
+#ifdef HVR_DEBUG_KNOBS
+  static const int dbg_wgs = std::getenv("HVR_BIGTILE_WGS") ? std::atoi(std::getenv("HVR_BIGTILE_WGS")) : -1;
+  if (dbg_wgs >= 0) nper = dbg_wgs;
+#endif
   const int grid = nper > 0 && tiles > nper ? nper : tiles;
   hipLaunchKernelGGL(kern, dim3(grid), dim3(BG_NT), lds, stream, p);
   return hipGetLastError();
 }
 
+static bool ring_routed(const GemmParams& p) {
+  if (p.dtype != DT_BF16 && p.dtype != DT_F16) return false;
+#ifdef HVR_DEBUG_KNOBS
+  static const int dbg_loop = std::getenv("HVR_BIGTILE_LOOP") ? std::atoi(std::getenv("HVR_BIGTILE_LOOP")) : -1;
+  if (dbg_loop >= 0) return dbg_loop != 0;
+#endif
+  return p.conv != 0 && p.KH * p.KW > 1 && p.N == BG_BN;
+}
+
 hipError_t run_bigtile(const GemmParams& p, hipStream_t stream) {
-  if (p.dtype == DT_F16S) return launch_bigtile<f16s_t, 9, 9>(p, stream);
-  if (p.dtype == DT_F16) return launch_bigtile<f16_t, 9, 9>(p, stream);
-  return launch_bigtile<bf16_t, 9, 9>(p, stream);
-}
-
-}
+  if (p.dtype == DT_F16S) return launch_bigtile<f16s_t, 9, 9, false>(p, stream);
+  const bool ring = p.tile_hint == kBigRing || (p.tile_hint != kBigForce && ring_routed(p));
+  if (p.dtype == DT_F16) return ring ? launch_bigtile<f16_t, 9, 9, true>(p, stream) : launch_bigtile<f16_t, 9, 9, false>(p, stream);
+  return ring ? launch_bigtile<bf16_t, 9, 9, true>(p, stream) : launch_bigtile<bf16_t, 9, 9, false>(p, stream);
+}
+
+}
diff --git a/hvrnet_amd/csrc/capi.hip b/hvrnet_amd/csrc/capi.hip
--- a/hvrnet_amd/csrc/capi.hip
+++ b/hvrnet_amd/csrc/capi.hip
@@ -201,7 +201,7 @@
   const int rc = gemm_params(d, p);
   if (rc) return rc;
   int hint = d->tile_hint;
-  if (hint == kBigForce) {
+  if (hint == kBigForce || hint == kBigRing) {
     if (!bigtile_supported(p, true)) return fail(HVR_EUNSUPPORTED, "the big-tile kernel takes bf16 products with N %% 256 == 0 and K %% 64 == 0");
     return check_launch(run_bigtile(p, (hipStream_t)stream), "hvr_gemm(big tile)");
   }
@@ -355,7 +355,7 @@
   p.alpha = d->alpha; p.beta = d->beta;
   if (pointwise) p.zero = d->zero;
   const int use_expand = expand_enabled();
-  if (p.tile_hint == kBigForce) {
+  if (p.tile_hint == kBigForce || p.tile_hint == kBigRing) {
     path = 0;
     return 0;
   }
@@ -391,7 +391,7 @@
   if (rc) return rc;
   if (path == 1) return check_launch(p.dtype == DT_F16S ? run_expand_split(p, (hipStream_t)stream) : run_expand(p, (hipStream_t)stream), "hvr_conv2d_nhwc(expand)");
   if (path == 2) return check_launch(run_conv3x3_c64(p, (hipStream_t)stream), "hvr_conv2d_nhwc(conv3x3_c64)");
-  if (path == 0 && d->tile_hint == kBigForce) {
+  if (path == 0 && (d->tile_hint == kBigForce || d->tile_hint == kBigRing)) {
     if (!bigtile_supported(p, true)) return fail(HVR_EUNSUPPORTED, "the big-tile kernel takes bf16 convs with Cout %% 256 == 0 and Cin %% 64 == 0");
     return check_launch(run_bigtile(p, (hipStream_t)stream), "hvr_conv2d_nhwc(big tile)");
   }
@@ -450,6 +450,21 @@
     return check_launch(run_tile_op(p, EPI_LINEAR, (hipStream_t)stream), "hvr_bottleneck_tail(tile engine)");
   }
   return fail(HVR_EUNSUPPORTED, "no fused tail kernel for C1=%d C2=%d Cout=%d", d->C1, d->C2, d->Cout);
+}
+
+int hvr_bottleneck_tail_hinted(const hvr_tail_desc* d, int tile_hint, void* stream) {
+  if (tile_hint == 0) return hvr_bottleneck_tail(d, stream);
+  GemmParams p;
+  const int rc = tail_params(d, p);
+  if (rc) return rc;
+  if (!tail_on_tile_engine(p)) return fail(HVR_EUNSUPPORTED, "no tile-engine form of the fused tail for C1=%d C2=%d Cout=%d", d->C1, d->C2, d->Cout);
+  p.tile_hint = tile_hint;
+  if (tile_hint == kBigForce || tile_hint == kBigRing) {
+    if (!bigtile_supported(p, false)) return fail(HVR_EUNSUPPORTED, "the big-tile kernel takes fused tails with Cout %% 256 == 0");
+    return check_launch(run_bigtile(p, (hipStream_t)stream), "hvr_bottleneck_tail_hinted(big tile)");
+  }
+  if (tile_hint < 0 || tile_hint > kNumTileShapes) return fail(HVR_EINVAL, "tile_hint %d is not a tile shape of the engine", tile_hint);
+  return check_launch(run_tile_op(p, EPI_LINEAR, (hipStream_t)stream), "hvr_bottleneck_tail_hinted(tile engine)");
 }
 
 static int tail_next_params(const hvr_tail_next_desc* d, GemmParams& p) {
diff --git a/hvrnet_amd/csrc/gemm_params.h b/hvrnet_amd/csrc/gemm_params.h
--- a/hvrnet_amd/csrc/gemm_params.h
+++ b/hvrnet_amd/csrc/gemm_params.h
@@ -75,6 +75,7 @@
 constexpr int kPcHint128 = kNumTileShapes + 2, kPcHint256 = kNumTileShapes + 3;
 bool pc_supported(const GemmParams& p, int epi);
 constexpr int kBigHint = kNumTileShapes + 4, kBigForce = kNumTileShapes + 5, kTwoLevelHint = kNumTileShapes + 6;
+constexpr int kBigRing = kNumTileShapes + 7;
 constexpr int kTwoLevelSteps = 8;
 bool bigtile_supported(const GemmParams& p, bool throughput);
 hipError_t run_bigtile(const GemmParams& p, hipStream_t stream);
diff --git a/hvrnet_amd/native.py b/hvrnet_amd/native.py
--- a/hvrnet_amd/native.py
+++ b/hvrnet_amd/native.py
@@ -94,6 +94,7 @@
     'hvr_conv2d_path': (_i, [ctypes.POINTER(ConvDesc)]),
     'hvr_conv2d_splitk_workspace_bytes': (_sz, [ctypes.POINTER(ConvDesc)]),
     'hvr_bottleneck_tail': (_i, [ctypes.POINTER(TailDesc), _vp]),
+    'hvr_bottleneck_tail_hinted': (_i, [ctypes.POINTER(TailDesc), _i, _vp]),
     'hvr_bottleneck_tail_supported': (_i, [ctypes.POINTER(TailDesc)]),
     'hvr_bottleneck_tail_next': (_i, [ctypes.POINTER(TailNextDesc), _vp]),
     'hvr_bottleneck_tail_next_supported': (_i, [ctypes.POINTER(TailNextDesc)]),
@@ -444,7 +445,7 @@
     return bool(lib().hvr_bottleneck_tail_supported(ctypes.byref(_tail_desc(h, x, w, bias, stride2, True, None))))
 
 
-def bottleneck_tail(h, x, w, bias, stride2=1, relu=True, out=None):
+def bottleneck_tail(h, x, w, bias, stride2=1, relu=True, out=None, tile=None):
     _need_cuda(h, x, w, bias)
     B, OH, OW, C1 = h.shape
     Cout = w.shape[0]
@@ -458,7 +459,10 @@
     if _prof is not None and _prof['detail']:
         tag = 'conv_expand tail %dx%d %d+%d->%d s%d' % (OH, OW, C1, x.shape[3], Cout, stride2)
     with _span(tag, work):
-        _check(lib().hvr_bottleneck_tail(ctypes.byref(d), _stream()), 'hvr_bottleneck_tail')
+        if tile:
+            _check(lib().hvr_bottleneck_tail_hinted(ctypes.byref(d), int(tile), _stream()), 'hvr_bottleneck_tail_hinted')
+        else:
+            _check(lib().hvr_bottleneck_tail(ctypes.byref(d), _stream()), 'hvr_bottleneck_tail')
     return y
 
 
@@ -625,6 +629,8 @@
 
 
 BIG_TILE_HINT = 16
+BIG_FORCE_HINT = 17
+BIG_RING_HINT = 19
 TWO_LEVEL_HINT = 18
 
 
diff --git a/include/hvr_hip.h b/include/hvr_hip.h
--- a/include/hvr_hip.h
+++ b/include/hvr_hip.h
@@ -70,6 +70,7 @@
   int32_t relu, dtype;
 } hvr_tail_desc;
 int hvr_bottleneck_tail(const hvr_tail_desc* d, void* stream);
+int hvr_bottleneck_tail_hinted(const hvr_tail_desc* d, int tile_hint, void* stream);
 int hvr_bottleneck_tail_supported(const hvr_tail_desc* d);
 
 typedef struct hvr_tail_next_desc {
```
